# slyforce/MusicStyleTransfer

Measured on AMD Instinct MI355X. Metric: piano-roll frames/s (VAE train step), higher is better.
Workload: dtype bf16; 1 GPU; BASELINE configs[1]: single-track piano-roll VAE train step, T=256, pitch=128, latent=64, batch=64/GPU, bf16; encoder 256x2x8h, decoder 128x1x8h (scripts/train-vae.sh), dropout 0.2; Xavier-initialised weights; global_batch=64, seq_len=256, pitches=128, latent=64, parallelism=dp1, params=1885440

## Files before the change

### include/mst_hip.h

```cpp
#ifndef MST_HIP_H
#define MST_HIP_H

#include <stdint.h>

#ifdef __cplusplus
extern "C" {
#endif

typedef void* mst_stream_t;

enum mst_status {
  MST_OK = 0,
  MST_ERR_INVALID = -1,
  MST_ERR_LAUNCH = -2,
  MST_ERR_UNSUPPORTED = -3
};

enum mst_dtype { MST_BF16 = 0, MST_F16 = 1, MST_F32 = 2 };

enum mst_act { MST_ACT_NONE = 0, MST_ACT_RELU = 1 };

int mst_version(void);
const char* mst_last_error(void);

// ... 7 lines not shown
int mst_event_record(void* ev, mst_stream_t stream);
int mst_event_sync(void* ev);
int mst_event_elapsed_ms(void* ev_start, void* ev_stop, float* ms_out);
int mst_event_destroy(void* ev);

typedef struct mst_gemm_args {
  int32_t dtype;
  int32_t c_f32;
  int64_t M, N, K;
  const void* A; int64_t lda;
  const void* B; int64_t ldb;
  void* C; int64_t ldc;
  const float* bias;
  const void* resid; int64_t ldr;
  int32_t act;
  const void* gate; int64_t ldg;
  float alpha;
  const float* rowadd; int64_t ldra; int64_t rowadd_period;
  const float* grpadd; int64_t ldga; const int32_t* grp_index;
  int64_t a_rows_per_group, a_group_stride, a_group_offset;
  int64_t c_rows_per_group, c_group_stride, c_group_offset;
  float dropout_p; uint64_t dropout_seed; uint32_t dropout_site;
  int32_t self_resid;
  const uint64_t* dropout_seed_ptr;
  int32_t a_u8;
  int32_t resid_phys;
} mst_gemm_args;

int mst_gemm_nt(const mst_gemm_args* args, mst_stream_t stream);
int mst_gemm_nt_form(const mst_gemm_args* args);

int mst_gemm_nt_pair(const mst_gemm_args* args0, const mst_gemm_args* args1, mst_stream_t stream);

typedef struct mst_bce_args {
  const uint8_t* labels;
  int64_t T;
  float label_smoothing;
  int32_t downweight;
  float* loss;
  void* probs; int64_t ldp;
  void* logits; int64_t ldl;
  float gscale;
} mst_bce_args;
int mst_gemm_sigmoid_bce(const mst_gemm_args* args, const mst_bce_args* bce, mst_stream_t stream);

typedef struct mst_ln_args {
  int32_t mode;
  const float* gamma;
  const float* beta;
  float eps;
  void* out; int64_t ld_out;
  float* mean; float* rstd;
  const void* x; int64_t ld_x;
  float* dgamma; float* dbeta;
  int32_t mask_mode;
  float* partials;
} mst_ln_args;

int mst_gemm_nt_ln(const mst_gemm_args* args, const mst_ln_args* ln, mst_stream_t stream);
int mst_gemm_sigmoid_bce_dgrad_ln(const mst_gemm_args* args, const mst_bce_args* bce, const mst_gemm_args* dgrad,
                                  const mst_ln_args* ln, mst_stream_t stream);
int64_t mst_gemm_nt_ln_parts(int64_t M);
int mst_gemm_sigmoid_bce_form(const mst_gemm_args* args, const mst_bce_args* bce, const mst_gemm_args* dgrad, const mst_ln_args* ln,
                              int64_t* form);

int mst_ffn_ln_fwd(const mst_gemm_args* ff1, const mst_gemm_args* ff2, const mst_ln_args* ln, mst_stream_t stream);
int mst_ffn_ln_bwd(const mst_gemm_args* ff2_dgrad, const mst_gemm_args* ff1_dgrad, const mst_ln_args* ln, mst_stream_t stream);
typedef struct mst_ln_bwd_in {
  const void* dy; int64_t ld_dy;
  const void* x;  int64_t ld_x;
  const float* gamma; const float* mean; const float* rstd;
  void* dx; int64_t ld_dx;
  void* dx_masked; int64_t ld_dxm;
  float* dgamma; float* dbeta; float* partials;
  int32_t mask_mode;
  float dropout_p; uint64_t dropout_seed; const uint64_t* dropout_seed_ptr; uint32_t dropout_site;
} mst_ln_bwd_in;
int mst_ffn_ln_bwd_lead(const mst_ln_bwd_in* lead, const mst_gemm_args* ff2_dgrad, const mst_gemm_args* ff1_dgrad,
                        const mst_ln_args* ln, mst_stream_t stream);
int mst_proj_ffn_ln_fwd(const mst_gemm_args* proj, const mst_ln_args* ln1, const mst_gemm_args* ff1, const mst_gemm_args* ff2,
                        const mst_ln_args* ln2, mst_stream_t stream);
int mst_dec_tail_step(const mst_gemm_args* proj, const mst_ln_args* ln1, const mst_gemm_args* ff1, const mst_gemm_args* ff2,
                      const mst_ln_args* ln3, const mst_gemm_args* out, const mst_bce_args* bce, const mst_gemm_args* out_dgrad,
                      const mst_ln_args* ln3_bwd, const mst_gemm_args* ff2_dgrad, const mst_gemm_args* ff1_dgrad,
                      const mst_ln_args* ln1_bwd, mst_stream_t stream);

typedef struct mst_partial_sum {
  const float* src; int64_t n_parts; int64_t stride; int64_t len;
  float* dst; float scale;
} mst_partial_sum;
int mst_partial_sums(const mst_partial_sum* jobs, int n, mst_stream_t stream);

typedef struct mst_wgrad_args {
  int32_t dtype;
  int64_t M, N, K;
  const void* A; int64_t lda;
  const void* B; int64_t ldb;
  float* dW; int64_t ldw;
  float* db;
  float scale;
  int64_t a_rows_per_group, a_group_stride, a_group_offset;
  int64_t b_rows_per_group, b_group_stride, b_group_offset;
  int32_t a_u8;
} mst_wgrad_args;

typedef struct mst_outer_job {
  const float* L; const void* R; int32_t r_dtype; int64_t r_stride;
  int64_t B, J, I;
  float* out; float* obias;
} mst_outer_job;
int mst_outer_jobs(const mst_outer_job* jobs, int n, mst_stream_t stream);
int mst_gemm_wgrad_batch_flush(const mst_wgrad_args* list, int n, float* scratch, int64_t scratch_bytes,
                               const mst_partial_sum* sums, int n_sums, const mst_outer_job* outers, int n_outers,
                               mst_stream_t stream);
int mst_gemm_wgrad_plan(const mst_wgrad_args* list, int n, int64_t scratch_bytes, int64_t* plan);

int mst_embed_fwd(int dtype, int64_t B, int64_t T, int64_t D,
                  const int32_t* tokens, const float* table, int64_t ldt,
                  const int32_t* classes, const float* cls_table, int64_t ldc,
                  const float* pos, int64_t ldp, float alpha,
                  void* out, int64_t ld_out, int64_t S_out, int64_t s_off,
                  uint8_t* keymask, mst_stream_t stream);

int mst_embed_bwd(int dtype, int64_t B, int64_t T, int64_t D,
                  const int32_t* tokens, float* dtable, int64_t ldt,
                  const int32_t* classes, float* dcls, int64_t ldc, float alpha,
                  const void* dX, int64_t ld_dx, int64_t S_out, int64_t s_off,
                  mst_stream_t stream);

int mst_group_colsum(int dtype, int64_t B, int64_t T, int64_t D, const void* X, int64_t ldx,
                     int64_t S_out, int64_t s_off, const int32_t* idx, float* dst, int64_t ldd,
                     float alpha, mst_stream_t stream);

int mst_mask_from_lengths(int64_t B, int64_t S, const int32_t* lens, int32_t add,
                          uint8_t* keymask, mst_stream_t stream);

int mst_attn_keysoftmax_fwd(int dtype, int64_t B, int64_t S, int64_t H, int64_t dh,
                            const void* qkv, int64_t ld_qkv, int64_t k_off, int64_t q_off, int64_t v_off,
                            const uint8_t* keymask, float* lse,
                            void* out, int64_t ld_out,
                            int64_t q_limit ,
                            mst_stream_t stream);

int mst_attn_qkv_fwd(int dtype, int64_t B, int64_t S, int64_t H, int64_t dh, const void* x, int64_t ld_x, const void* w,
                     int64_t ld_w, const float* bias, void* qkv, int64_t ld_qkv, int64_t k_off, int64_t q_off, int64_t v_off,
                     const uint8_t* keymask, float* lse, void* out, int64_t ld_out, int64_t q_limit, mst_stream_t stream);
int mst_attn_keysoftmax_bwd(int dtype, int64_t B, int64_t S, int64_t H, int64_t dh,
                            const void* qkv, int64_t ld_qkv, int64_t k_off, int64_t q_off, int64_t v_off,
                            const uint8_t* keymask, const float* lse,
                            const void* dout, int64_t ld_dout,
                            void* dqkv, int64_t ld_dqkv, float* delta,
                            int64_t q_limit ,
                            mst_stream_t stream);

int mst_attn_fwd_form(int dtype, int64_t B, int64_t S, int64_t H, int64_t dh, int64_t ld_qkv, int64_t k_off, int64_t q_off,
                      int64_t v_off, int64_t ld_out, int64_t q_limit, int fused, int64_t ld_x, int64_t ld_w, int64_t* form);
int mst_attn_bwd_form(int dtype, int64_t B, int64_t S, int64_t H, int64_t dh, int64_t ld_qkv, int64_t k_off, int64_t q_off,
                      int64_t v_off, int64_t ld_dout, int64_t ld_dqkv, int64_t q_limit, int64_t* form);

int mst_attn_causal_fwd(int dtype, int64_t B, int64_t S, int64_t H, int64_t dh,
                        const void* qkv, int64_t ld_qkv, int64_t k_off, int64_t q_off, int64_t v_off,
                        const uint8_t* keymask, float* lse, void* out, int64_t ld_out, mst_stream_t stream);
int mst_attn_causal_bwd(int dtype, int64_t B, int64_t S, int64_t H, int64_t dh,
                        const void* qkv, int64_t ld_qkv, int64_t k_off, int64_t q_off, int64_t v_off,
                        const uint8_t* keymask, const float* lse, const void* dout, int64_t ld_dout,
                        void* dqkv, int64_t ld_dqkv, float* delta, mst_stream_t stream);

int mst_layernorm_fwd(int dtype, int64_t M, int64_t D, const void* x, int64_t ldx,
                      const float* gamma, const float* beta, float eps,
                      void* y, int64_t ldy, float* mean, float* rstd,
                      int64_t row_id_stride ,
                      mst_stream_t stream);

int mst_layernorm_bwd(int dtype, int64_t M, int64_t D, const void* x, int64_t ldx,
                      const float* gamma, const float* mean, const float* rstd,
                      const void* dy, int64_t ldy, void* dx, int64_t ld_dx,
                      void* dx_masked, int64_t ld_dxm, float* dgamma, float* dbeta,
                      int mask_mode, float dropout_p, uint64_t dropout_seed, uint32_t dropout_site,
                      const uint64_t* dropout_seed_ptr,
                      int64_t row_id_stride ,
                      float* partials ,
                      mst_stream_t stream);
int64_t mst_layernorm_bwd_parts(int64_t M, int64_t D);

int mst_latent_fwd(int dtype, int64_t B, int64_t De, int64_t Z, int64_t Dd,
                   const void* enc_out, int64_t enc_sample_stride,
                   const float* Wl, const float* bl, const float* eps,
                   const float* Wh, const float* bh,
                   const int32_t* classes, const float* cls_d, int64_t ld_cls,
                   const float* pos_d, float alpha_d,
                   float* mu, float* sigma, float* z, float* kl,
                   void* dec_in, int64_t dec_sample_stride, mst_stream_t stream);
int mst_latent_fwd_proj(int dtype, int64_t B, int64_t De, int64_t Z, int64_t Dd,
                        const void* enc_out, int64_t enc_sample_stride,
                        const float* Wl, const float* bl, const float* eps,
                        const float* Wh, const float* bh,
                        const int32_t* classes, const float* cls_d, int64_t ld_cls,
                        const float* pos_d, float alpha_d,
                        float* mu, float* sigma, float* z, float* kl,
                        void* dec_in, int64_t dec_sample_stride,
                        const void* Wq, int64_t ld_wq, const float* bq, void* qkv0, int64_t qkv_sample_stride, int64_t nq,
                        mst_stream_t stream);
int mst_latent_rows(int dtype, int64_t N, int64_t M, int64_t Z, int64_t Dd,
                    const float* zsrc, const float* ssrc, const int32_t* a, const int32_t* b, const float* w, int mode,
                    float tau, uint64_t seed, const uint64_t* seed_ptr, uint32_t site, int64_t row0,
                    const float* Wh, const float* bh,
                    const int32_t* ca, const int32_t* cb, const float* cw, const float* cls_d, int64_t ld_cls, int64_t n_classes,
                    const float* pos_d, float alpha_d,
                    float* z_out, void* dec_in, int64_t dec_stride, mst_stream_t stream);

int mst_latent_bwd_vec(int dtype, int64_t B, int64_t De, int64_t Z, int64_t Dd, const float* Wl, const float* eps, const float* Wh,
                       const int32_t* classes, const float* mu, const float* sigma, const void* d_dec_in, int64_t dec_sample_stride,
                       float alpha_d, float kl_weight, float gscale, float enc_scale, float* dcls_d, int64_t ld_cls,
                       void* d_enc_out, int64_t denc_sample_stride, float* scratch, mst_stream_t stream);
int mst_latent_bwd_vec_proj(int dtype, int64_t B, int64_t De, int64_t Z, int64_t Dd, const float* Wl, const float* eps, const float* Wh,
                            const int32_t* classes, const float* mu, const float* sigma,
                            const void* dq0, int64_t dq_sample_stride, const void* Wt, int64_t ld_wt, int64_t nq,
                            const void* resid0, int64_t resid_sample_stride,
                            float alpha_d, float kl_weight, float gscale, float enc_scale, float* dcls_d, int64_t ld_cls,
                            void* d_enc_out, int64_t denc_sample_stride, float* scratch, mst_stream_t stream);

int mst_latent_bwd_vec_sched(int dtype, int64_t B, int64_t De, int64_t Z, int64_t Dd, const float* Wl, const float* eps, const float* Wh,
                             const int32_t* classes, const float* mu, const float* sigma, const void* d_dec_in, int64_t dec_sample_stride,
                             float alpha_d, const float* sched, const float* kl, float gscale, float enc_scale, float* dcls_d,
                             int64_t ld_cls, void* d_enc_out, int64_t denc_sample_stride, float* scratch, mst_stream_t stream);
int mst_latent_bwd_vec_proj_sched(int dtype, int64_t B, int64_t De, int64_t Z, int64_t Dd, const float* Wl, const float* eps,
                                  const float* Wh, const int32_t* classes, const float* mu, const float* sigma,
                                  const void* dq0, int64_t dq_sample_stride, const void* Wt, int64_t ld_wt, int64_t nq,
                                  const void* resid0, int64_t resid_sample_stride,
                                  float alpha_d, const float* sched, const float* kl, float gscale, float enc_scale, float* dcls_d,
                                  int64_t ld_cls, void* d_enc_out, int64_t denc_sample_stride, float* scratch, mst_stream_t stream);

int mst_latent_form(int64_t De, int64_t Z, int64_t Dd, int64_t nq, const void* Wl, int64_t* form);

int mst_reparam_kl_fwd(int64_t B, int64_t Z, const float* mu, const float* sigma, const float* eps,
                       float* z, float* kl, mst_stream_t stream);
int mst_reparam_kl_bwd(int64_t B, int64_t Z, const float* mu, const float* sigma, const float* eps,
                       const float* dz, float kl_weight, float* dmu, float* dsigma, mst_stream_t stream);

typedef struct mst_row_tail_args {
  int32_t dtype;
  int64_t B, D;
  const void* att; int64_t rs_att;
  const void* resid; int64_t rs_res;
  const void* Wp; int64_t ldwp; const float* bp;
  const float* g1; const float* be1;
  const void* W1; int64_t ldw1; const float* b1;
  const void* W2; int64_t ldw2; const float* b2;
  const float* g2; const float* be2;
  void* h1; void* x1; void* h2; void* x2; int64_t rs_d;
  void* a; int64_t rs_a;
  float* mean1; float* rstd1; float* mean2; float* rstd2; int64_t stat_stride;
  float eps;
  float dropout_p; uint64_t dropout_seed; const uint64_t* dropout_seed_ptr; uint32_t site0;
  int64_t phys_stride;
  uint32_t* sync;
  uint32_t* status;
} mst_row_tail_args;
int mst_row_tail_fwd(const mst_row_tail_args* args, mst_stream_t stream);
int mst_row_tail_fwd_ride(const mst_row_tail_args* args, const mst_gemm_args* rider, uint32_t* queue, mst_stream_t stream);
int mst_row_tail_fwd_ride_shadows(const mst_row_tail_args* args, const mst_gemm_args* rider, uint32_t* queue, int sh_dtype,
                                  const float* sh_w, void* sh_wt16, const int64_t* sh_desc, const int64_t* sh_prefix, int64_t sh_n_mat,
                                  int64_t sh_tiles, mst_stream_t stream);
typedef struct mst_row_tail_bwd_args {
  int32_t dtype;
  int64_t B, D;
  const void* dy; int64_t rs_dy;
  const void* h2; const void* h1; int64_t rs_d;
  const void* a; int64_t rs_a;
  const float* mean1; const float* rstd1; const float* mean2; const float* rstd2; int64_t stat_stride;
  const float* g1; const float* g2;
  const void* W2t; int64_t ldw2t;
  const void* W1t; int64_t ldw1t;
  const void* Wpt; int64_t ldwpt;
  void* dh; void* dhm; void* dx1; void* dh1m; int64_t rs_c;
  void* dpre; int64_t rs_dpre;
  void* dh1; int64_t rs_dh1;
  void* datt; int64_t rs_datt;
  float* dg1; float* db1; float* dg2; float* db2;
  float dropout_p; uint64_t dropout_seed; const uint64_t* dropout_seed_ptr; uint32_t site0;
  int64_t phys_stride;
  uint32_t* sync;
  uint32_t* status;
} mst_row_tail_bwd_args;
int mst_row_tail_bwd(const mst_row_tail_bwd_args* args, mst_stream_t stream);
int mst_row_tail_bwd_ride(const mst_row_tail_bwd_args* args, const mst_gemm_args* rider, uint32_t* queue, mst_stream_t stream);
int mst_row_tail_form(int backward, int dtype, int64_t D, const mst_gemm_args* rider, int64_t sh_tiles, int64_t* form);

int mst_attn_decode(int dtype, int64_t B, int64_t H, int64_t dh, int64_t n_keys, int64_t t_max, const void* cache,
                    int64_t ld, int64_t k_off, int64_t q_off, int64_t v_off, int mode, void* out, int64_t ld_out,
                    mst_stream_t stream);

int mst_beam_step(int64_t B, int64_t K, int64_t V, int64_t i, int64_t L, const float* probs, int64_t ldp, const float* scores_in,
                  float* scores_out, const int32_t* seqs_in, int32_t* seqs_out, int32_t* hyp_src, int32_t* word, int32_t* active,
                  int32_t eos, int32_t pad, mst_stream_t stream);
int mst_beam_gather(const void* in, void* out, const int32_t* src, int64_t N, int64_t n_rows, int64_t row_bytes, int64_t t_max,
                    mst_stream_t stream);
int mst_beam_gather_cols(const void* in, void* out, const int32_t* src, int64_t N, int64_t n_rows, int64_t row_bytes, int64_t t_max,
                         int64_t skip_begin, int64_t skip_bytes, mst_stream_t stream);
int mst_sample_step(int64_t N, int64_t V, int64_t i, int64_t L, const float* probs, int64_t ldp, int32_t* seqs, float* scores,
                    int32_t* word, int32_t* active, uint64_t seed, int32_t eos, int32_t pad, mst_stream_t stream);
int mst_frame_step(int dtype, int64_t N, int64_t P, int64_t i, int64_t L, const void* logits, int64_t ldl, float tau, int mode, float thr,
                   const uint64_t* seed_ptr, uint8_t* frames, int64_t ldf, uint8_t* roll, int64_t ldr, float* scores, float* probs_out,
                   mst_stream_t stream);
int mst_token_step(int dtype, int64_t N, int64_t V, int64_t i, int64_t L, const void* logits, int64_t ldl, float tau, int32_t top_k,
                   float top_p, const uint64_t* seed_ptr, int32_t* seqs, float* scores, int32_t* word, int32_t* active,
// ... 106 lines not shown
```

### musicstyletransfer_amd/csrc/attention.hip

```cpp
#include <math.h>
#include <stdlib.h>
#include <type_traits>
#include "common.hpp"

namespace mst {

constexpr int ATT_STAGE = 64;
template <int DH> struct LdsLd { static constexpr int V = DH + 8; };
constexpr int ATT_WG_ROWS = 128;
constexpr float MASK_VALUE = -1e9f;
constexpr float NEG_BIG = -3.0e38f;
constexpr float LOG2E = 1.4426950408889634f;

__device__ __forceinline__ void key_consts(bool in_range, bool valid_key, float rmax, float logl, float scale, float& sk2,
                                           float& ck2) {
  if (!in_range) { sk2 = 0.f; ck2 = -INFINITY; }
  else if (!valid_key) { sk2 = 0.f; ck2 = -logl * LOG2E; }
  else { sk2 = scale * LOG2E; ck2 = -(rmax + logl) * LOG2E; }
}
__device__ __forceinline__ float fast_exp2(float x) { return __builtin_amdgcn_exp2f(x); }
#define MST_FOR_TILES(kt, bits) for (uint64_t mst_m_ = (bits); mst_m_; mst_m_ &= mst_m_ - 1) if (const int kt = __builtin_ctzll(mst_m_); true)
__device__ __forceinline__ uint64_t tile_bits(int n) { return n >= 64 ? ~0ull : ((1ull << n) - 1ull); }
__device__ __forceinline__ uint64_t padded_tile_mask(const float* sSk, const float* sCk, int n_tiles, int lane) {
  uint32_t lo = 0u, hi = 0u;
// ... 887 lines not shown
        a.lse[plane + bh * S + k_lane] = logl;
      }
      key_consts(in, vk, in ? M : 0.f, in ? logl : 0.f, a.scale, sSk[k_lane], sCk[k_lane]);
      sMadd[k_lane] = madd; sMax[k_lane] = in ? M : 0.f; sLogl[k_lane] = in ? logl : INFINITY;
    }
    padded |= (in && !vk);
  }
  if constexpr (DH <= 16) {
    if (lone) {
      const int64_t e = S - 1;
      const bool vk = a.keymask[b * S + e];
      const float madd = vk ? 0.f : MASK_VALUE;
      float ke[DH];
      if (restage) {
#pragma unroll
        for (int f = 0; f < DH; ++f) ke[f] = to_f32(base[a.k_off + e * a.ld_qkv + f]);
      } else {
        lds_row_load<T, DH>(sK + e * LD, ke);
      }
      float m = NEG_BIG, l = 0.f;
      for (int q = tid; q < S; q += nthr) {
        const float t = fmaf(lds_row_dot<T, DH>(sQ + q * LD, ke), a.scale, madd);
        const float m_new = fmaxf(m, t);
        l = l * __expf(m - m_new) + __expf(t - m_new);
        m = m_new;
      }
      const float mw = wave_max(m);
      const float lw = wave_sum(l * __expf(m - mw));
      if (lane == 0) { sRed[wave] = mw; sRed[16 + wave] = lw; }
      __syncthreads();
      if (tid == 0) {
        float M = NEG_BIG, L = 0.f;
        for (int w = 0; w < NW; ++w) M = fmaxf(M, sRed[w]);
        for (int w = 0; w < NW; ++w) L += sRed[16 + w] * __expf(sRed[w] - M);
        const float logl = __logf(L);
        a.lse[bh * S + e] = M;
        a.lse[plane + bh * S + e] = logl;
        key_consts(true, vk, M, logl, a.scale, sSk[e], sCk[e]);
        sMadd[e] = madd; sMax[e] = M; sLogl[e] = logl;
        for (int k = (int)S; k < SP; ++k) { key_consts(false, false, 0.f, 0.f, a.scale, sSk[k], sCk[k]); sMadd[k] = MASK_VALUE; sMax[k] = 0.f; sLogl[k] = INFINITY; }
      }
      padded |= !vk;
    }
  }
  const bool exact = __syncthreads_or(padded);
  const uint64_t pad_tiles = exact ? padded_tile_mask(sSk, sCk, NB, lane) : 0ull;
  ATT_STAMP(3);
  if constexpr (CHUNKED) {
    constexpr int OBM = 2;
    typename Act<T>::vec8 qf[OBM][KS];
    f32x16 o[OBM][DB];
    bool act[OBM];
#pragma unroll
    for (int i = 0; i < OBM; ++i) {
      const int ob = wave + i * NW;
      act[i] = ob < NBo && (int64_t)ob * 32 < a.q_limit;
#pragma unroll
      for (int s = 0; s < KS; ++s) qf[i][s] = glb_row_frag<T>(base + a.q_off, a.ld_qkv, act[i] ? (int64_t)ob * 32 + (lane & 31) : S, S, s, lane);
#pragma unroll
      for (int d = 0; d < DB; ++d) o[i][d] = zero16<DH>();
    }
    const int tiles_c = CR / 32;
    for (int c = 0; c < a.restage; ++c) {
      if (c > 0) __syncthreads();
      const int64_t k0 = (int64_t)c * CR;
      stage_pair<T, DH>(sK, base + a.k_off + k0 * a.ld_qkv, a.ld_qkv, S - k0, sV, base + a.v_off + k0 * a.ld_qkv, a.ld_qkv, S - k0, CR, tid, nthr);
      __syncthreads();
      const int nt = (NBo - c * tiles_c) < tiles_c ? (NBo - c * tiles_c) : tiles_c;
#pragma unroll
      for (int i = 0; i < OBM; ++i) {
        if (!act[i]) continue;
        if (exact) {
          const uint64_t padc = (pad_tiles >> (c * tiles_c)) & tile_bits(nt);
          MST_FOR_TILES(kt, ~padc & tile_bits(nt)) fwd_out_tile<T, DH, false>(sK, sV, sSk + k0, sCk + k0, sMadd + k0, sMax + k0, sLogl + k0, kt, a.scale, qf[i], o[i], lane);
          MST_FOR_TILES(kt, padc) fwd_out_tile<T, DH, true>(sK, sV, sSk + k0, sCk + k0, sMadd + k0, sMax + k0, sLogl + k0, kt, a.scale, qf[i], o[i], lane);
        } else {
          for (int kt = 0; kt < nt; ++kt) fwd_out_tile<T, DH, false>(sK, sV, sSk + k0, sCk + k0, sMadd + k0, sMax + k0, sLogl + k0, kt, a.scale, qf[i], o[i], lane);
        }
      }
    }
    T* og = reinterpret_cast<T*>(a.out) + b * S * a.ld_out + hd * DH;
#pragma unroll
    for (int i = 0; i < OBM; ++i) {
      const int64_t q_lane = (int64_t)(wave + i * NW) * 32 + (lane & 31);
      owner_store<T, DH>((act[i] && q_lane < S && q_lane < a.q_limit) ? og + q_lane * a.ld_out : nullptr, o[i], lane);
    }
    return;
  }
  if (restage) {
    stage_pair<T, DH>(sK, base + a.k_off, a.ld_qkv, S, sV, base + a.v_off, a.ld_qkv, S, SP, tid, nthr);
    __syncthreads();
  }

  for (int ob = wave; ob < NBo; ob += NW) {
    if ((int64_t)ob * 32 >= a.q_limit) break;
    typename Act<T>::vec8 qf[KS];
#pragma unroll
    for (int s = 0; s < KS; ++s)
      qf[s] = restage ? glb_row_frag<T>(base + a.q_off, a.ld_qkv, (int64_t)ob * 32 + (lane & 31), S, s, lane) : lds_row_frag<T, DH>(sQ, ob * 32, s, lane);
    f32x16 o[DB];
#pragma unroll
    for (int d = 0; d < DB; ++d) o[d] = zero16<DH>();
    if (exact) {
      MST_FOR_TILES(kt, ~pad_tiles & tile_bits(NBo)) fwd_out_tile<T, DH, false>(sK, sV, sSk, sCk, sMadd, sMax, sLogl, kt, a.scale, qf, o, lane);
      MST_FOR_TILES(kt, pad_tiles & tile_bits(NBo)) fwd_out_tile<T, DH, true>(sK, sV, sSk, sCk, sMadd, sMax, sLogl, kt, a.scale, qf, o, lane);
    } else {
      for (int kt = 0; kt < NBo; ++kt) fwd_out_tile<T, DH, false>(sK, sV, sSk, sCk, sMadd, sMax, sLogl, kt, a.scale, qf, o, lane);
    }
    if constexpr (DH <= 16) {
      if (lone) {
        if (exact) fwd_out_tile<T, DH, true, true>(sK, sV, sSk, sCk, sMadd, sMax, sLogl, NB - 1, a.scale, qf, o, lane);
        else fwd_out_tile<T, DH, false, true>(sK, sV, sSk, sCk, sMadd, sMax, sLogl, NB - 1, a.scale, qf, o, lane);
      }
    }
    T* og = reinterpret_cast<T*>(a.out) + b * S * a.ld_out + hd * DH;
    const int64_t q_lane = ob * 32 + (lane & 31);
    owner_store<T, DH>((q_lane < S && q_lane < a.q_limit) ? og + q_lane * a.ld_out : nullptr, o, lane);
  }
  ATT_STAMP(4);
  if constexpr (DH <= 16) {
    if (lone) {
      const int64_t e = S - 1;
      float qe[DH], acc[DH];
      if (restage) {
#pragma unroll
        for (int f = 0; f < DH; ++f) qe[f] = to_f32(base[a.q_off + e * a.ld_qkv + f]);
      } else {
        lds_row_load<T, DH>(sQ + e * LD, qe);
      }
#pragma unroll
      for (int f = 0; f < DH; ++f) acc[f] = 0.f;
      for (int k = tid; k < S; k += nthr) {
        const float x = lds_row_dot<T, DH>(sK + k * LD, qe);
        const float p = exact ? exact_prob(x, a.scale, sMadd[k], sMax[k], sLogl[k]) : fast_exp2(fmaf(x, sSk[k], sCk[k]));
        lds_row_axpy<T, DH>(p, sV + k * LD, acc);
      }
#pragma unroll
      for (int f = 0; f < DH; ++f) acc[f] = wave_sum(acc[f]);
      if (lane == 0) {
#pragma unroll
        for (int f = 0; f < DH; ++f) sRed[wave * DH + f] = acc[f];
      }
      __syncthreads();
      if (tid < DH) {
        float o_e = 0.f;
        for (int w = 0; w < NW; ++w) o_e += sRed[w * DH + tid];
        T* og = reinterpret_cast<T*>(a.out) + b * S * a.ld_out + hd * DH;
        og[e * a.ld_out + tid] = (T)o_e;
      }
    }
  }
}

template <typename T, int DH, bool SPARSE>
__global__ __launch_bounds__(RES_MAX_WAVES<DH> * 64) __attribute__((amdgpu_waves_per_eu(DH == 16 ? ATT16_WAVES : (DH == 64 ? 2 : 4)))) void attn_bwd_res_kernel(AttnArgs a) {
  constexpr int KS = DH / 16, DB = (DH + 31) / 32, LD = LdsLd<DH>::V;
  extern __shared__ __attribute__((aligned(16))) unsigned char att_smem[];
  const int64_t S = a.S;
  const int NB = (int)((S + 31) / 32), SP = NB * 32;
  T* bufA = reinterpret_cast<T*>(att_smem);
  T* bufB = bufA + SP * LD;
  float* sSk = reinterpret_cast<float*>(bufB + SP * LD);
  float* sCk = sSk + SP; float* sMadd = sCk + SP; float* sMax = sMadd + SP; float* sLogl = sMax + SP; float* sNd = sLogl + SP;
  float* sRed = sNd + SP;
  const int tid = threadIdx.x, lane = tid & 63, wave = tid >> 6, nthr = blockDim.x, NW = nthr >> 6;
  const int64_t bh = res_wg_bh(a.B, a.H), b = (int64_t)((uint32_t)bh / (uint32_t)a.H), hd = bh - b * a.H;
  const int64_t plane = a.B * a.H * S;
  const bool lone = !SPARSE && lone_row_shape(S, DH);
  const int NBo = lone ? NB - 1 : NB;
  const float log2_scale = __log2f(a.scale);
  const T* base = reinterpret_cast<const T*>(a.qkv) + b * S * a.ld_qkv + hd * DH;
  const T* Kg = base + a.k_off;
  const T* Qg = base + a.q_off;
  const T* Vg = base + a.v_off;
  const T* dOg = reinterpret_cast<const T*>(a.dout) + b * S * a.ld_dout + hd * DH;
  T* dbase = reinterpret_cast<T*>(a.dqkv) + b * S * a.ld_dqkv + hd * DH;
  constexpr bool sparse = SPARSE;
  const int64_t do_rows = sparse ? a.q_limit : S;
  typename Act<T>::vec8 kf[KS], vf[KS];
#pragma unroll
  for (int s = 0; s < KS; ++s) {
    kf[s] = glb_row_frag<T>(Kg, a.ld_qkv, wave * 32 + (lane & 31), S, s, lane);
    vf[s] = glb_row_frag<T>(Vg, a.ld_qkv, wave * 32 + (lane & 31), S, s, lane);
  }
  ATT_STAMP(0);
  stage_pair<T, DH>(bufA, Qg, a.ld_qkv, S, bufB, dOg, a.ld_dout, do_rows, SP, tid, nthr);
  __syncthreads();
  ATT_STAMP(1);
  const int nq0 = sparse ? 1 : NBo;

  int padded = 0;
  for (int ob = wave; ob < NBo; ob += NW) {
    const int64_t k_lane = ob * 32 + (lane & 31);
    if (ob != wave) {
#pragma unroll
      for (int s = 0; s < KS; ++s) {
        kf[s] = glb_row_frag<T>(Kg, a.ld_qkv, k_lane, S, s, lane);
        vf[s] = glb_row_frag<T>(Vg, a.ld_qkv, k_lane, S, s, lane);
      }
    }
    const bool in = k_lane < S;
    const bool vk = in && a.keymask[b * S + k_lane];
    const float rmax = in ? a.lse[bh * S + k_lane] : 0.f;
    const float logl = in ? a.lse[plane + bh * S + k_lane] : INFINITY;
    const float madd = vk ? 0.f : MASK_VALUE;
    float sk2, ck2;
    key_consts(in, vk, rmax, in ? logl : 0.f, a.scale, sk2, ck2);
    const float ck2s = ck2 + log2_scale;
    const bool exact_w = __any(in && !vk);
    padded |= (in && !vk);
    f32x16 acc[DB];
    float neg_delta = 0.f;
    T* const drow = in ? dbase + k_lane * a.ld_dqkv : nullptr;
#pragma unroll
    for (int d = 0; d < DB; ++d) acc[d] = zero16<DH>();
    if (exact_w) for (int qt = 0; qt < nq0; ++qt) bwd_kv_tile<T, DH, 0, true>(bufA, bufB, qt, a.scale, kf, vf, sk2, ck2, madd, rmax, logl, neg_delta, acc, lane);
    else for (int qt = 0; qt < nq0; ++qt) bwd_kv_tile<T, DH, 0, false>(bufA, bufB, qt, a.scale, kf, vf, sk2, ck2, madd, rmax, logl, neg_delta, acc, lane);
    if constexpr (DH <= 16 && !SPARSE) {
      if (lone) {
        if (exact_w) bwd_kv_tile<T, DH, 0, true, false, true>(bufA, bufB, NB - 1, a.scale, kf, vf, sk2, ck2, madd, rmax, logl, neg_delta, acc, lane);
        else bwd_kv_tile<T, DH, 0, false, false, true>(bufA, bufB, NB - 1, a.scale, kf, vf, sk2, ck2, madd, rmax, logl, neg_delta, acc, lane);
      }
    }
    {
      const float delta = delta_from_dv<T, DH>(acc, vf, lane);
      if (lane < 32 && in) a.delta[bh * S + k_lane] = delta;
      neg_delta = -delta;
    }
    owner_store<T, DH>(drow ? drow + a.v_off : nullptr, acc, lane);
    ATT_STAMP(2);
#pragma unroll
    for (int d = 0; d < DB; ++d) acc[d] = zero16<DH>();
    if (exact_w) for (int qt = 0; qt < nq0; ++qt) bwd_kv_tile<T, DH, 1, true>(bufA, bufB, qt, a.scale, kf, vf, sk2, ck2s, madd, rmax, logl, neg_delta, acc, lane);
    else for (int qt = 0; qt < nq0; ++qt) bwd_kv_tile<T, DH, 1, false>(bufA, bufB, qt, a.scale, kf, vf, sk2, ck2s, madd, rmax, logl, neg_delta, acc, lane);
    if (sparse) {
      if (exact_w) for (int qt = nq0; qt < NB; ++qt) bwd_kv_tile<T, DH, 1, true, true>(bufA, bufB, qt, a.scale, kf, vf, sk2, ck2s, madd, rmax, logl, neg_delta, acc, lane);
      else for (int qt = nq0; qt < NB; ++qt) bwd_kv_tile<T, DH, 1, false, true>(bufA, bufB, qt, a.scale, kf, vf, sk2, ck2s, madd, rmax, logl, neg_delta, acc, lane);
    }
    if constexpr (DH <= 16 && !SPARSE) {
      if (lone) {
        if (exact_w) bwd_kv_tile<T, DH, 1, true, false, true>(bufA, bufB, NB - 1, a.scale, kf, vf, sk2, ck2s, madd, rmax, logl, neg_delta, acc, lane);
        else bwd_kv_tile<T, DH, 1, false, false, true>(bufA, bufB, NB - 1, a.scale, kf, vf, sk2, ck2s, madd, rmax, logl, neg_delta, acc, lane);
      }
    }
    owner_store<T, DH>(drow ? drow + a.k_off : nullptr, acc, lane);
    if (lane < 32) {
      sSk[k_lane] = sk2; sCk[k_lane] = ck2s; sMadd[k_lane] = madd; sMax[k_lane] = rmax; sLogl[k_lane] = logl;
      sNd[k_lane] = in ? neg_delta : 0.f;
    }
  }
  if constexpr (DH <= 16 && !SPARSE) {
    if (lone) {
      const int64_t e = S - 1;
      float ke[DH], ve[DH], acc[DH];
#pragma unroll
      for (int f = 0; f < DH; ++f) { ke[f] = to_f32(Kg[e * a.ld_qkv + f]); ve[f] = to_f32(Vg[e * a.ld_qkv + f]); }
      const bool vk = a.keymask[b * S + e];
      const float rmax = a.lse[bh * S + e], logl = a.lse[plane + bh * S + e], madd = vk ? 0.f : MASK_VALUE;
      float sk2, ck2;
      key_consts(true, vk, rmax, logl, a.scale, sk2, ck2);
      const float ck2s = ck2 + log2_scale;
      padded |= !vk;
#pragma unroll
      for (int f = 0; f < DH; ++f) acc[f] = 0.f;
      for (int q = tid; q < S; q += nthr) {
        const float x = lds_row_dot<T, DH>(bufA + q * LD, ke);
        const float pr = vk ? fast_exp2(fmaf(x, sk2, ck2)) : exact_prob(x, a.scale, madd, rmax, logl);
        lds_row_axpy<T, DH>(pr, bufB + q * LD, acc);
      }
#pragma unroll
      for (int f = 0; f < DH; ++f) acc[f] = wave_sum(acc[f]);
      if (lane == 0) {
#pragma unroll
        for (int f = 0; f < DH; ++f) sRed[wave * DH + f] = acc[f];
      }
      __syncthreads();
      if (tid < DH) {
        float dv = 0.f;
        for (int w = 0; w < NW; ++w) dv += sRed[w * DH + tid];
        sRed[LONE_RED / 2 + tid] = dv;
        dbase[e * a.ld_dqkv + a.v_off + tid] = (T)dv;
      }
      __syncthreads();
      float delta = 0.f;
#pragma unroll
      for (int f = 0; f < DH; ++f) delta = fmaf(ve[f], sRed[LONE_RED / 2 + f], delta);
#pragma unroll
      for (int f = 0; f < DH; ++f) acc[f] = 0.f;
      for (int q = tid; q < S; q += nthr) {
        const float x = lds_row_dot<T, DH>(bufA + q * LD, ke);
        const float ps = vk ? fast_exp2(fmaf(x, sk2, ck2s)) : exact_prob(x, a.scale, madd, rmax, logl) * a.scale;
        const float dl = ps * (lds_row_dot<T, DH>(bufB + q * LD, ve) - delta);
        lds_row_axpy<T, DH>(dl, bufA + q * LD, acc);
      }
#pragma unroll
      for (int f = 0; f < DH; ++f) acc[f] = wave_sum(acc[f]);
      __syncthreads();
      if (lane == 0) {
#pragma unroll
        for (int f = 0; f < DH; ++f) sRed[wave * DH + f] = acc[f];
      }
      __syncthreads();
      if (tid < DH) {
        float dk = 0.f;
        for (int w = 0; w < NW; ++w) dk += sRed[w * DH + tid];
        dbase[e * a.ld_dqkv + a.k_off + tid] = (T)dk;
      }
      if (tid == 0) {
        a.delta[bh * S + e] = delta;
        sSk[e] = sk2; sCk[e] = ck2s; sMadd[e] = madd; sMax[e] = rmax; sLogl[e] = logl; sNd[e] = -delta;
        for (int k = (int)S; k < SP; ++k) {
          float s0, c0;
          key_consts(false, false, 0.f, 0.f, a.scale, s0, c0);
          sSk[k] = s0; sCk[k] = c0 + log2_scale; sMadd[k] = MASK_VALUE; sMax[k] = 0.f; sLogl[k] = INFINITY; sNd[k] = 0.f;
        }
      }
    }
  }
  ATT_STAMP(3);
  typename Act<T>::vec8 qf[KS], dof[KS];
#pragma unroll
  for (int s = 0; s < KS; ++s) {
    qf[s] = glb_row_frag<T>(Qg, a.ld_qkv, wave * 32 + (lane & 31), S, s, lane);
    dof[s] = glb_row_frag<T>(dOg, a.ld_dout, wave * 32 + (lane & 31), do_rows, s, lane);
  }
  __syncthreads();
  stage_pair<T, DH>(bufA, Kg, a.ld_qkv, S, bufB, Vg, a.ld_qkv, S, SP, tid, nthr);
  const bool exact = __syncthreads_or(padded);
  const uint64_t pad_tiles = exact ? padded_tile_mask(sSk, sCk, NB, lane) : 0ull;
  ATT_STAMP(4);

  for (int ob = wave; ob < NBo; ob += NW) {
    const int64_t q_lane = ob * 32 + (lane & 31);
    if (ob != wave) {
#pragma unroll
      for (int s = 0; s < KS; ++s) {
        qf[s] = glb_row_frag<T>(Qg, a.ld_qkv, q_lane, S, s, lane);
        dof[s] = glb_row_frag<T>(dOg, a.ld_dout, q_lane, do_rows, s, lane);
      }
    }
    f32x16 acc[DB];
#pragma unroll
    for (int d = 0; d < DB; ++d) acc[d] = zero16<DH>();
    if (sparse && ob > 0) {
      if (exact) {
        MST_FOR_TILES(kt, ~pad_tiles & tile_bits(NB)) bwd_q_tile<T, DH, false, true>(bufA, bufB, sSk, sCk, sMadd, sMax, sLogl, sNd, kt, a.scale, qf, dof, acc, lane);
        MST_FOR_TILES(kt, pad_tiles & tile_bits(NB)) bwd_q_tile<T, DH, true, true>(bufA, bufB, sSk, sCk, sMadd, sMax, sLogl, sNd, kt, a.scale, qf, dof, acc, lane);
      } else for (int kt = 0; kt < NB; ++kt) bwd_q_tile<T, DH, false, true>(bufA, bufB, sSk, sCk, sMadd, sMax, sLogl, sNd, kt, a.scale, qf, dof, acc, lane);
    } else if (exact) {
      MST_FOR_TILES(kt, ~pad_tiles & tile_bits(NBo)) bwd_q_tile<T, DH, false>(bufA, bufB, sSk, sCk, sMadd, sMax, sLogl, sNd, kt, a.scale, qf, dof, acc, lane);
      MST_FOR_TILES(kt, pad_tiles & tile_bits(NBo)) bwd_q_tile<T, DH, true>(bufA, bufB, sSk, sCk, sMadd, sMax, sLogl, sNd, kt, a.scale, qf, dof, acc, lane);
    } else {
      for (int kt = 0; kt < NBo; ++kt) bwd_q_tile<T, DH, false>(bufA, bufB, sSk, sCk, sMadd, sMax, sLogl, sNd, kt, a.scale, qf, dof, acc, lane);
    }
    if constexpr (DH <= 16 && !SPARSE) {
      if (lone) {
        if (exact) bwd_q_tile<T, DH, true, false, true>(bufA, bufB, sSk, sCk, sMadd, sMax, sLogl, sNd, NB - 1, a.scale, qf, dof, acc, lane);
        else bwd_q_tile<T, DH, false, false, true>(bufA, bufB, sSk, sCk, sMadd, sMax, sLogl, sNd, NB - 1, a.scale, qf, dof, acc, lane);
      }
    }
    owner_store<T, DH>(q_lane < S ? dbase + a.q_off + q_lane * a.ld_dqkv : nullptr, acc, lane);
  }
  ATT_STAMP(5);
  if constexpr (DH <= 16 && !SPARSE) {
    if (lone) {
      const int64_t e = S - 1;
      float qe[DH], doe[DH], acc[DH];
#pragma unroll
      for (int f = 0; f < DH; ++f) { qe[f] = to_f32(Qg[e * a.ld_qkv + f]); doe[f] = to_f32(dOg[e * a.ld_dout + f]); acc[f] = 0.f; }
      for (int k = tid; k < S; k += nthr) {
        const float x = lds_row_dot<T, DH>(bufA + k * LD, qe);
        const float ps = exact ? exact_prob(x, a.scale, sMadd[k], sMax[k], sLogl[k]) * a.scale : fast_exp2(fmaf(x, sSk[k], sCk[k]));
        const float dl = ps * (lds_row_dot<T, DH>(bufB + k * LD, doe) + sNd[k]);
        lds_row_axpy<T, DH>(dl, bufA + k * LD, acc);
      }
#pragma unroll
      for (int f = 0; f < DH; ++f) acc[f] = wave_sum(acc[f]);
      if (lane == 0) {
#pragma unroll
        for (int f = 0; f < DH; ++f) sRed[wave * DH + f] = acc[f];
      }
      __syncthreads();
      if (tid < DH) {
        float dq = 0.f;
        for (int w = 0; w < NW; ++w) dq += sRed[w * DH + tid];
        dbase[e * a.ld_dqkv + a.q_off + tid] = (T)dq;
      }
    }
  }
}

template <typename T, int DH, int OBM>
__global__ __launch_bounds__(512) void attn_bwd_q_chunk_kernel(AttnArgs a, int n_chunks) {
  constexpr int KS = DH / 16, DB = (DH + 31) / 32, LD = LdsLd<DH>::V;
  extern __shared__ __attribute__((aligned(16))) unsigned char att_smem[];
  const int64_t S = a.S;
  const int NB = (int)((S + 31) / 32), SP = NB * 32, CR = SP / n_chunks;
  T* sK = reinterpret_cast<T*>(att_smem);
  T* sV = sK + CR * LD;
  float* sSk = reinterpret_cast<float*>(sV + CR * LD);
  float* sCk = sSk + SP; float* sMadd = sCk + SP; float* sMax = sMadd + SP; float* sLogl = sMax + SP; float* sNd = sLogl + SP;
  const int tid = threadIdx.x, lane = tid & 63, wave = tid >> 6, nthr = blockDim.x, NW = nthr >> 6;
  const int64_t bh = res_wg_bh(a.B, a.H), b = (int64_t)((uint32_t)bh / (uint32_t)a.H), hd = bh - b * a.H;
  const int64_t plane = a.B * a.H * S;
  const float log2_scale = __log2f(a.scale);
  const T* base = reinterpret_cast<const T*>(a.qkv) + b * S * a.ld_qkv + hd * DH;
  const T* dOg = reinterpret_cast<const T*>(a.dout) + b * S * a.ld_dout + hd * DH;
  const bool sparse = a.q_limit > 0 && a.q_limit <= 32;
  const int64_t do_rows = sparse ? a.q_limit : S;
  typename Act<T>::vec8 qf[OBM][KS], dof[OBM][KS];
  f32x16 acc[OBM][DB];
  bool act[OBM];
#pragma unroll
  for (int i = 0; i < OBM; ++i) {
    const int ob = wave + i * NW;
    act[i] = ob < NB;
    const int64_t q_lane = act[i] ? (int64_t)ob * 32 + (lane & 31) : S;
#pragma unroll
    for (int s = 0; s < KS; ++s) {
      qf[i][s] = glb_row_frag<T>(base + a.q_off, a.ld_qkv, q_lane, S, s, lane);
      dof[i][s] = glb_row_frag<T>(dOg, a.ld_dout, q_lane, do_rows, s, lane);
    }
#pragma unroll
    for (int d = 0; d < DB; ++d) acc[i][d] = zero16<DH>();
  }
  int padded = 0;
  for (int k = tid; k < SP; k += nthr) {
    const bool in = k < S;
    const bool vk = in && a.keymask[b * S + k];
    const float rmax = in ? a.lse[bh * S + k] : 0.f, logl = in ? a.lse[plane + bh * S + k] : 0.f;
    float sk2, ck2;
    key_consts(in, vk, rmax, logl, a.scale, sk2, ck2);
    sSk[k] = sk2; sCk[k] = ck2 + log2_scale;
    sMadd[k] = vk ? 0.f : MASK_VALUE; sMax[k] = rmax; sLogl[k] = in ? logl : INFINITY;
    sNd[k] = in ? -a.delta[bh * S + k] : 0.f;
    padded |= (in && !vk);
  }
  const bool exact = __syncthreads_or(padded);
  const uint64_t pad_tiles = exact ? padded_tile_mask(sSk, sCk, NB, lane) : 0ull;
  const int tiles_c = CR / 32;
  for (int c = 0; c < n_chunks; ++c) {
    if (c > 0) __syncthreads();
    const int64_t k0 = (int64_t)c * CR;
    if (k0 >= S) break;
    stage_pair<T, DH>(sK, base + a.k_off + k0 * a.ld_qkv, a.ld_qkv, S - k0, sV, base + a.v_off + k0 * a.ld_qkv, a.ld_qkv, S - k0, CR, tid, nthr);
    __syncthreads();
    const int nt = (NB - c * tiles_c) < tiles_c ? (NB - c * tiles_c) : tiles_c;
#pragma unroll
    for (int i = 0; i < OBM; ++i) {
      if (!act[i]) continue;
      const bool light = sparse && (wave + i * NW) > 0;
      if (light) {
        if (exact) {
          const uint64_t padc = (pad_tiles >> (c * tiles_c)) & tile_bits(nt);
          MST_FOR_TILES(kt, ~padc & tile_bits(nt)) bwd_q_tile<T, DH, false, true>(sK, sV, sSk + k0, sCk + k0, sMadd + k0, sMax + k0, sLogl + k0, sNd + k0, kt, a.scale, qf[i], dof[i], acc[i], lane);
          MST_FOR_TILES(kt, padc) bwd_q_tile<T, DH, true, true>(sK, sV, sSk + k0, sCk + k0, sMadd + k0, sMax + k0, sLogl + k0, sNd + k0, kt, a.scale, qf[i], dof[i], acc[i], lane);
        } else for (int kt = 0; kt < nt; ++kt) bwd_q_tile<T, DH, false, true>(sK, sV, sSk + k0, sCk + k0, sMadd + k0, sMax + k0, sLogl + k0, sNd + k0, kt, a.scale, qf[i], dof[i], acc[i], lane);
      } else if (exact) {
        const uint64_t padc = (pad_tiles >> (c * tiles_c)) & tile_bits(nt);
        MST_FOR_TILES(kt, ~padc & tile_bits(nt)) bwd_q_tile<T, DH, false>(sK, sV, sSk + k0, sCk + k0, sMadd + k0, sMax + k0, sLogl + k0, sNd + k0, kt, a.scale, qf[i], dof[i], acc[i], lane);
        MST_FOR_TILES(kt, padc) bwd_q_tile<T, DH, true>(sK, sV, sSk + k0, sCk + k0, sMadd + k0, sMax + k0, sLogl + k0, sNd + k0, kt, a.scale, qf[i], dof[i], acc[i], lane);
      } else {
        for (int kt = 0; kt < nt; ++kt) bwd_q_tile<T, DH, false>(sK, sV, sSk + k0, sCk + k0, sMadd + k0, sMax + k0, sLogl + k0, sNd + k0, kt, a.scale, qf[i], dof[i], acc[i], lane);
      }
    }
  }
  T* dst = reinterpret_cast<T*>(a.dqkv) + b * S * a.ld_dqkv + hd * DH + a.q_off;
#pragma unroll
  for (int i = 0; i < OBM; ++i) {
    const int64_t q_lane = (int64_t)(wave + i * NW) * 32 + (lane & 31);
    owner_store<T, DH>((act[i] && q_lane < S) ? dst + q_lane * a.ld_dqkv : nullptr, acc[i], lane);
  }
}

static int choose_resident(int64_t S, int64_t n_wg, size_t lds_bytes, int waves_cu = 16, bool lone = false, int max_nw = 16) {
  const char* force = getenv("MST_ATTN_PATH");
  if (force && force[0] == 's') return 0;
  const size_t LDS_CU = 160 * 1024;
  if (lds_bytes > LDS_CU - 1024) return 0;
  const int NB = (int)cdiv(S, 32) - (lone ? 1 : 0);
  const int by_grid = (int)cdiv(n_wg, 256);
  int best = 0;
  double best_score = 0.0;
  for (int nw = 1; nw <= max_nw && nw <= NB; ++nw) {
    int wgs = waves_cu / nw;
    if ((size_t)wgs * lds_bytes > LDS_CU) wgs = (int)(LDS_CU / lds_bytes);
    if (wgs > by_grid) wgs = by_grid;
    if (wgs < 1) continue;
    const double eff = (double)NB / (double)(nw * cdiv(NB, nw));
    const double score = (double)(wgs * nw) * eff;
    if (score >= best_score) { best_score = score; best = nw; }
  }
  return best;
}
static size_t res_lds_fwd(int dh, int64_t S, int tiles) { const size_t SP = (size_t)cdiv(S, 32) * 32; return (size_t)tiles * SP * (dh + 8) * 2 + 5 * SP * 4 + LONE_RED * 4; }
static size_t res_lds_bwd(int dh, int64_t S) { const size_t SP = (size_t)cdiv(S, 32) * 32; return 2 * SP * (dh + 8) * 2 + 6 * SP * 4 + LONE_RED * 4; }
static int res_max_waves(int dh) { return dh == 64 ? RES_MAX_WAVES<64> : RES_MAX_WAVES<32>; }

static int attn_check(int64_t B, int64_t S, int64_t H, int64_t dh, int64_t ld, int64_t k_off, int64_t q_off, int64_t v_off) {
  MST_CHECK_ARG(B > 0 && S > 0 && H > 0, "attention: B,S,H must be positive");
  MST_CHECK_ARG(dh == 16 || dh == 32 || dh == 64, "attention: head size must be 16, 32 or 64 (got %lld)", (long long)dh);
  MST_CHECK_ARG(ld % 8 == 0 && k_off % 8 == 0 && q_off % 8 == 0 && v_off % 8 == 0, "attention: ld and offsets must be multiples of 8");
  MST_CHECK_ARG(B * H <= 65535, "attention: B*H too large for grid.y");
  return MST_OK;
}
static int attn_check_fwd(int64_t B, int64_t S, int64_t H, int64_t dh, int64_t ld_qkv, int64_t k_off, int64_t q_off, int64_t v_off, int64_t ld_out) {
  const int rc = attn_check(B, S, H, dh, ld_qkv, k_off, q_off, v_off);
  if (rc) return rc;
  MST_CHECK_ARG(ld_out >= H * dh, "mst_attn_keysoftmax_fwd: ld_out < H*dh");
  return MST_OK;
}
static int attn_check_qkv(int64_t B, int64_t S, int64_t H, int64_t dh, int64_t ld_x, int64_t ld_w, int64_t ld_qkv, int64_t k_off, int64_t q_off,
                          int64_t v_off, int64_t ld_out) {
  const int rc = attn_check(B, S, H, dh, ld_qkv, k_off, q_off, v_off);
  if (rc) return rc;
  const int64_t Dm = H * dh;
  MST_CHECK_ARG(ld_x % 8 == 0 && ld_x >= Dm && ld_w % 8 == 0 && ld_w >= Dm && ld_qkv >= 3 * Dm && ld_out >= Dm,
                "mst_attn_qkv_fwd: leading dimensions must be multiples of 8 and cover the model width");
  MST_CHECK_ARG(k_off + Dm <= 3 * Dm && q_off + Dm <= 3 * Dm && v_off + Dm <= 3 * Dm, "mst_attn_qkv_fwd: section offsets beyond the 3 D weight rows");
  return MST_OK;
}
static int attn_check_bwd(int64_t B, int64_t S, int64_t H, int64_t dh, int64_t ld_qkv, int64_t k_off, int64_t q_off, int64_t v_off, int64_t ld_dout,
                          int64_t ld_dqkv) {
  const int rc = attn_check(B, S, H, dh, ld_qkv, k_off, q_off, v_off);
  if (rc) return rc;
  MST_CHECK_ARG(ld_dout % 8 == 0 && ld_dout >= H * dh && ld_dqkv % 8 == 0, "mst_attn_keysoftmax_bwd: bad leading dims");
  return MST_OK;
}
static int check_act_dtype(int dtype) { return dispatch_act(dtype, [](auto) -> int { return MST_OK; }); }
static int64_t fwd_q_limit(int64_t q_limit, int64_t S) { return (q_limit > 0 && q_limit < S) ? q_limit : S; }
static int64_t bwd_q_limit(int64_t q_limit, int64_t S) { return (q_limit > 0 && q_limit < S) ? q_limit : 0; }

enum { ATT_FWD_RES3 = 0, ATT_FWD_RES2 = 1, ATT_FWD_CHUNKED = 2, ATT_FWD_FUSED = 3, ATT_FWD_STREAM = 4 };
enum { ATT_BWD_RES = 0, ATT_BWD_STREAM_CHUNKQ = 1, ATT_BWD_STREAM = 2 };
struct AttnFwdForm { int path, waves; size_t lds; int lone, restage; int64_t grid_stats, grid_out; };
struct AttnBwdForm { int path, waves; size_t lds; int sparse, lone, dq_chunks, dq_waves; };
constexpr int ATT_DQ_OBM = 4, ATT_DQ_NW = 8;

static AttnFwdForm attn_fwd_form(int dh, int64_t S, int64_t H, int64_t n_wg, int64_t q_limit, bool fused_call) {
  AttnFwdForm f = {};
  const int NB = (int)cdiv(S, 32);
  if (fused_call && dh == 32) {
    const int64_t Dm = H * dh;
    const size_t lds = res_lds_fwd(32, S, 3);
    const int nw = choose_resident(S, n_wg, lds, 16, false);
    if (nw >= NB && nw >= 6 && Dm % QKV_KC == 0) { f.path = ATT_FWD_FUSED; f.waves = nw; f.lds = lds; return f; }
  }
  const bool lone = lone_row_shape(S, dh) && q_limit >= S;
  const int waves_cu = dh == 16 ? 4 * ATT16_WAVES : 16;
  f.lone = lone;
  for (int tiles = 3; tiles >= 2; --tiles) {
    const size_t lds = res_lds_fwd(dh, S, tiles);
    if (const int nw = choose_resident(S, n_wg, lds, waves_cu, lone)) {
      f.path = tiles == 3 ? ATT_FWD_RES3 : ATT_FWD_RES2; f.waves = nw; f.lds = lds; f.restage = tiles == 3 ? 0 : 1;
      return f;
    }
  }
  if (!lone && dh >= 32 && NB % 2 == 0) {
    const size_t lds = res_lds_fwd(dh, S, 1);
    const int maxw = res_max_waves(dh);
    const int nw = choose_resident(S, n_wg, lds, maxw, false, maxw);
    if (nw && NB <= 2 * nw) { f.path = ATT_FWD_CHUNKED; f.waves = nw; f.lds = lds; f.restage = 2; return f; }
  }
  f.path = ATT_FWD_STREAM; f.waves = 4; f.lone = 0;
  f.grid_stats = cdiv(S, ATT_WG_ROWS); f.grid_out = cdiv(q_limit, ATT_WG_ROWS);
  return f;
}
static AttnBwdForm attn_bwd_form(int dh, int64_t S, int64_t n_wg, int64_t q_limit) {
  AttnBwdForm f = {};
  f.sparse = q_limit > 0 && q_limit <= 32;
  const bool lone = lone_row_shape(S, dh) && !f.sparse;
  const size_t lds = res_lds_bwd(dh, S);
  if (const int nw = choose_resident(S, n_wg, lds, dh == 16 ? 4 * ATT16_WAVES : res_max_waves(dh), lone, res_max_waves(dh))) {
    f.path = ATT_BWD_RES; f.waves = nw; f.lds = lds; f.lone = lone;
    return f;
  }
  f.path = ATT_BWD_STREAM; f.waves = 4;
  const int NB = (int)cdiv(S, 32);
  if (dh == 32 && NB <= ATT_DQ_OBM * ATT_DQ_NW) {
    for (int nc = 1; nc <= 4; nc *= 2) {
      if (NB % nc != 0) break;
      const size_t lds_q = (size_t)2 * (NB * 32 / nc) * (dh + 8) * 2 + (size_t)6 * NB * 32 * 4;
      if (lds_q > 150 * 1024) continue;
      f.path = ATT_BWD_STREAM_CHUNKQ; f.lds = lds_q; f.dq_chunks = nc; f.dq_waves = ATT_DQ_NW;
      break;
    }
  }
  return f;
}

template <typename T, int DH>
static int launch_fwd(const AttnArgs& a_in, const AttnFwdForm& f, hipStream_t s) {
  AttnArgs a = a_in;
  a.restage = f.restage;
  const dim3 grid_res((unsigned)(a.B * a.H)), block_res(f.waves * 64);
  switch (f.path) {
    case ATT_FWD_FUSED: {
      if constexpr (DH == 32) {
        static size_t granted = 64 * 1024;
        if (const int rc = lds_opt_in(reinterpret_cast<const void*>(&attn_fwd_res_kernel<T, DH, true>), f.lds, &granted, "attn_fwd_res_kernel (fused projection)")) return rc;
        hipLaunchKernelGGL((attn_fwd_res_kernel<T, DH, true>), grid_res, block_res, f.lds, s, a);
        MST_CHECK_LAUNCH("attn_fwd_res_kernel (fused projection)");
        return MST_OK;
      }
      break;
    }
    case ATT_FWD_CHUNKED: {
      if (DH >= 32) {
        static size_t granted = 64 * 1024;
        if (const int rc = lds_opt_in(reinterpret_cast<const void*>(&attn_fwd_res_kernel<T, DH, false, true>), f.lds, &granted, "attn_fwd_res_kernel (chunked)")) return rc;
        hipLaunchKernelGGL((attn_fwd_res_kernel<T, DH, false, true>), grid_res, block_res, f.lds, s, a);
        MST_CHECK_LAUNCH("attn_fwd_res_kernel (chunked)");
        return MST_OK;
      }
      break;
    }
    case ATT_FWD_RES3:
    case ATT_FWD_RES2: {
      static size_t granted = 64 * 1024;
      if (const int rc = lds_opt_in(reinterpret_cast<const void*>(&attn_fwd_res_kernel<T, DH>), f.lds, &granted, "attn_fwd_res_kernel")) return rc;
      hipLaunchKernelGGL((attn_fwd_res_kernel<T, DH>), grid_res, block_res, f.lds, s, a);
      MST_CHECK_LAUNCH("attn_fwd_res_kernel");
      return MST_OK;
    }
    case ATT_FWD_STREAM: {
      const dim3 grid((unsigned)f.grid_stats, (unsigned)(a.B * a.H));
      hipLaunchKernelGGL((attn_fwd_stats_kernel<T, DH>), grid, dim3(256), 0, s, a);
      MST_CHECK_LAUNCH("attn_fwd_stats_kernel");
      const dim3 grid_o((unsigned)f.grid_out, (unsigned)(a.B * a.H));
      hipLaunchKernelGGL((attn_fwd_out_kernel<T, DH>), grid_o, dim3(256), 0, s, a);
      MST_CHECK_LAUNCH("attn_fwd_out_kernel");
      return MST_OK;
    }
  }
  set_error("attention forward: form %d has no kernel at head size %d", f.path, DH);
  return MST_ERR_INVALID;
}
template <typename T, int DH>
static int launch_bwd(const AttnArgs& a, const AttnBwdForm& f, hipStream_t s) {
  if (f.path == ATT_BWD_RES) {
    static size_t granted[2] = {64 * 1024, 64 * 1024};
    const void* fn = f.sparse ? reinterpret_cast<const void*>(&attn_bwd_res_kernel<T, DH, true>)
                              : reinterpret_cast<const void*>(&attn_bwd_res_kernel<T, DH, false>);
    if (const int rc = lds_opt_in(fn, f.lds, &granted[f.sparse], "attn_bwd_res_kernel")) return rc;
    if (f.sparse) hipLaunchKernelGGL((attn_bwd_res_kernel<T, DH, true>), dim3((unsigned)(a.B * a.H)), dim3(f.waves * 64), f.lds, s, a);
    else hipLaunchKernelGGL((attn_bwd_res_kernel<T, DH, false>), dim3((unsigned)(a.B * a.H)), dim3(f.waves * 64), f.lds, s, a);
    MST_CHECK_LAUNCH("attn_bwd_res_kernel");
    return MST_OK;
  }
  const dim3 grid((unsigned)cdiv(a.S, ATT_WG_ROWS), (unsigned)(a.B * a.H));
  if (f.sparse) hipLaunchKernelGGL((attn_bwd_kv_kernel<T, DH, true>), grid, dim3(256), 0, s, a);
  else hipLaunchKernelGGL((attn_bwd_kv_kernel<T, DH, false>), grid, dim3(256), 0, s, a);
  MST_CHECK_LAUNCH("attn_bwd_kv_kernel");
  if (f.path == ATT_BWD_STREAM_CHUNKQ) {
    if (DH == 32) {
      static size_t granted = 64 * 1024;
      if (const int rc = lds_opt_in(reinterpret_cast<const void*>(&attn_bwd_q_chunk_kernel<T, DH, ATT_DQ_OBM>), f.lds, &granted, "attn_bwd_q_chunk_kernel")) return rc;
      hipLaunchKernelGGL((attn_bwd_q_chunk_kernel<T, DH, ATT_DQ_OBM>), dim3((unsigned)(a.B * a.H)), dim3(f.dq_waves * 64), f.lds, s, a, f.dq_chunks);
      MST_CHECK_LAUNCH("attn_bwd_q_chunk_kernel");
      return MST_OK;
    }
    set_error("attention backward: chunked dQ has no kernel at head size %d", DH);
    return MST_ERR_INVALID;
  }
  hipLaunchKernelGGL((attn_bwd_q_kernel<T, DH>), grid, dim3(256), 0, s, a);
  MST_CHECK_LAUNCH("attn_bwd_q_kernel");
  return MST_OK;
}
template <typename T>
static int launch_fwd_dh(int64_t dh, const AttnArgs& a, const AttnFwdForm& f, hipStream_t s) {
  if (dh == 16) return launch_fwd<T, 16>(a, f, s);
  if (dh == 32) return launch_fwd<T, 32>(a, f, s);
  return launch_fwd<T, 64>(a, f, s);
}


template <typename T, int DH>
__global__ __launch_bounds__(64) void attn_decode_kernel(int64_t H, int64_t n_keys, int64_t t_max, const T* __restrict__ cache,
                                                          int64_t ld, int64_t k_off, int64_t q_off, int64_t v_off, int mode,
                                                          float scale, T* __restrict__ out, int64_t ld_out) {
  const int64_t b = blockIdx.x / H, hd = blockIdx.x % H;
  const int lane = threadIdx.x;
  const T* base = cache + b * t_max * ld + hd * DH;
  float q[DH];
#pragma unroll
  for (int d = 0; d < DH; ++d) q[d] = to_f32(base[(n_keys - 1) * ld + q_off + d]);
  float m = -INFINITY;
  if (mode == 1) {
    for (int64_t k = lane; k < n_keys; k += 64) {
      float l = 0.f;
#pragma unroll
      for (int d = 0; d < DH; ++d) l = fmaf(to_f32(base[k * ld + k_off + d]), q[d], l);
      m = fmaxf(m, l * scale);
    }
    m = wave_max(m);
  }
  float acc[DH], z = 0.f;
#pragma unroll
  for (int d = 0; d < DH; ++d) acc[d] = 0.f;
  for (int64_t k = lane; k < n_keys; k += 64) {
    float p = 1.f;
    if (mode == 1) {
      float l = 0.f;
#pragma unroll
      for (int d = 0; d < DH; ++d) l = fmaf(to_f32(base[k * ld + k_off + d]), q[d], l);
      p = __expf(l * scale - m);
    }
    z += p;
#pragma unroll
    for (int d = 0; d < DH; ++d) acc[d] = fmaf(p, to_f32(base[k * ld + v_off + d]), acc[d]);
  }
  z = wave_sum(z);
  const float inv = (mode == 1) ? 1.f / z : 1.f;
#pragma unroll
  for (int d = 0; d < DH; ++d) {
    const float v = wave_sum(acc[d]);
    if (lane == 0) out[b * ld_out + hd * DH + d] = from_f32<T>(v * inv);
  }
}

}

using namespace mst;

extern "C" int mst_attn_keysoftmax_fwd(int dtype, int64_t B, int64_t S, int64_t H, int64_t dh, const void* qkv,
                                       int64_t ld_qkv, int64_t k_off, int64_t q_off, int64_t v_off,
                                       const uint8_t* keymask, float* lse, void* out, int64_t ld_out,
                                       int64_t q_limit, mst_stream_t stream) {
  int rc = attn_check(B, S, H, dh, ld_qkv, k_off, q_off, v_off);
  if (rc) return rc;
  MST_CHECK_ARG(qkv && keymask && lse && out, "mst_attn_keysoftmax_fwd: null pointer");
  rc = attn_check_fwd(B, S, H, dh, ld_qkv, k_off, q_off, v_off, ld_out);
  if (rc) return rc;
  AttnArgs a = {};
  a.B = B; a.S = S; a.H = H; a.qkv = qkv; a.ld_qkv = ld_qkv; a.k_off = k_off; a.q_off = q_off; a.v_off = v_off;
  a.keymask = keymask; a.lse = lse; a.out = out; a.ld_out = ld_out;
  a.q_limit = fwd_q_limit(q_limit, S);
  a.scale = 1.f / sqrtf((float)dh);
  hipStream_t s = (hipStream_t)stream;
  return dispatch_act(dtype, [&](auto tag) -> int {
    return launch_fwd_dh<decltype(tag)>(dh, a, attn_fwd_form((int)dh, S, H, B * H, a.q_limit, false), s);
  });
}

static void put_fwd_form(const AttnFwdForm& f, int64_t* form) {
  const int64_t v[8] = {f.path, f.waves, (int64_t)f.lds, f.lone, f.grid_stats, f.grid_out, 0, 0};
  for (int i = 0; i < 8; ++i) form[i] = v[i];
}
extern "C" int mst_attn_fwd_form(int dtype, int64_t B, int64_t S, int64_t H, int64_t dh, int64_t ld_qkv, int64_t k_off, int64_t q_off,
                                 int64_t v_off, int64_t ld_out, int64_t q_limit, int fused, int64_t ld_x, int64_t ld_w, int64_t* form) {
  MST_CHECK_ARG(form != nullptr, "mst_attn_fwd_form: null form");
  int rc = fused ? attn_check_qkv(B, S, H, dh, ld_x, ld_w, ld_qkv, k_off, q_off, v_off, ld_out)
                 : attn_check_fwd(B, S, H, dh, ld_qkv, k_off, q_off, v_off, ld_out);
  if (rc == MST_OK) rc = check_act_dtype(dtype);
  if (rc) return rc;
  put_fwd_form(attn_fwd_form((int)dh, S, H, B * H, fwd_q_limit(q_limit, S), fused != 0), form);
  return MST_OK;
}
extern "C" int mst_attn_bwd_form(int dtype, int64_t B, int64_t S, int64_t H, int64_t dh, int64_t ld_qkv, int64_t k_off, int64_t q_off,
                                 int64_t v_off, int64_t ld_dout, int64_t ld_dqkv, int64_t q_limit, int64_t* form) {
  MST_CHECK_ARG(form != nullptr, "mst_attn_bwd_form: null form");
  int rc = attn_check_bwd(B, S, H, dh, ld_qkv, k_off, q_off, v_off, ld_dout, ld_dqkv);
  if (rc == MST_OK) rc = check_act_dtype(dtype);
  if (rc) return rc;
  const AttnBwdForm f = attn_bwd_form((int)dh, S, B * H, bwd_q_limit(q_limit, S));
  const int64_t v[8] = {f.path, f.waves, (int64_t)f.lds, f.sparse, f.lone, f.dq_chunks, f.dq_waves, 0};
  for (int i = 0; i < 8; ++i) form[i] = v[i];
  return MST_OK;
}

#ifdef MST_ATT_STAMPS
extern "C" int mst_debug_att_loop(uint64_t* host_out) {
  return hipMemcpyFromSymbol(host_out, HIP_SYMBOL(mst::g_att_loop), sizeof(uint64_t) * 256) == hipSuccess ? 0 : -1;
}
extern "C" int mst_debug_att_stamps(uint64_t* host_out) {
  return hipMemcpyFromSymbol(host_out, HIP_SYMBOL(mst::g_att_stamps), sizeof(uint64_t) * 8192) == hipSuccess ? 0 : -1;
}
#endif

extern "C" int mst_attn_qkv_fwd(int dtype, int64_t B, int64_t S, int64_t H, int64_t dh, const void* x, int64_t ld_x, const void* w,
                                int64_t ld_w, const float* bias, void* qkv, int64_t ld_qkv, int64_t k_off, int64_t q_off, int64_t v_off,
                                const uint8_t* keymask, float* lse, void* out, int64_t ld_out, int64_t q_limit, mst_stream_t stream) {
  int rc = attn_check_qkv(B, S, H, dh, ld_x, ld_w, ld_qkv, k_off, q_off, v_off, ld_out);
  if (rc) return rc;
  const int64_t Dm = H * dh;
  MST_CHECK_ARG(x && w && bias && qkv && keymask && lse && out, "mst_attn_qkv_fwd: null pointer");
  MST_CHECK_ARG(((uintptr_t)x % 16 == 0) && ((uintptr_t)w % 16 == 0) && ((uintptr_t)bias % 16 == 0) && ((uintptr_t)qkv % 16 == 0),
                "mst_attn_qkv_fwd: operands must be 16-byte aligned");
  rc = check_act_dtype(dtype);
  if (rc) return rc;
  AttnArgs a = {};
  a.B = B; a.S = S; a.H = H; a.qkv = qkv; a.ld_qkv = ld_qkv; a.k_off = k_off; a.q_off = q_off; a.v_off = v_off;
  a.keymask = keymask; a.lse = lse; a.out = out; a.ld_out = ld_out;
  a.q_limit = fwd_q_limit(q_limit, S);
  a.scale = 1.f / sqrtf((float)dh);
  const AttnFwdForm f = attn_fwd_form((int)dh, S, H, B * H, a.q_limit, true);
  if (f.path == ATT_FWD_FUSED) {
    a.x = x; a.ld_x = ld_x; a.w = w; a.ld_w = ld_w; a.bias = bias; a.Dm = Dm;
  } else {
    mst_gemm_args g = {};
    g.dtype = dtype; g.M = B * S; g.N = 3 * Dm; g.K = Dm;
    g.A = x; g.lda = ld_x; g.B = w; g.ldb = ld_w; g.C = qkv; g.ldc = ld_qkv; g.bias = bias; g.alpha = 1.f;
    rc = mst_gemm_nt(&g, stream);
    if (rc) return rc;
  }
  hipStream_t s = (hipStream_t)stream;
  return dispatch_act(dtype, [&](auto tag) -> int { return launch_fwd_dh<decltype(tag)>(dh, a, f, s); });
}

extern "C" int mst_attn_keysoftmax_bwd(int dtype, int64_t B, int64_t S, int64_t H, int64_t dh, const void* qkv,
                                       int64_t ld_qkv, int64_t k_off, int64_t q_off, int64_t v_off,
                                       const uint8_t* keymask, const float* lse, const void* dout, int64_t ld_dout,
                                       void* dqkv, int64_t ld_dqkv, float* delta, int64_t q_limit, mst_stream_t stream) {
  int rc = attn_check(B, S, H, dh, ld_qkv, k_off, q_off, v_off);
  if (rc) return rc;
  MST_CHECK_ARG(qkv && keymask && lse && dout && dqkv && delta, "mst_attn_keysoftmax_bwd: null pointer");
  rc = attn_check_bwd(B, S, H, dh, ld_qkv, k_off, q_off, v_off, ld_dout, ld_dqkv);
  if (rc) return rc;
  AttnArgs a = {};
  a.B = B; a.S = S; a.H = H; a.qkv = qkv; a.ld_qkv = ld_qkv; a.k_off = k_off; a.q_off = q_off; a.v_off = v_off;
  a.keymask = keymask; a.lse = const_cast<float*>(lse); a.dout = dout; a.ld_dout = ld_dout; a.dqkv = dqkv;
  a.ld_dqkv = ld_dqkv; a.delta = delta;
  a.q_limit = bwd_q_limit(q_limit, S);
  a.scale = 1.f / sqrtf((float)dh);
  hipStream_t s = (hipStream_t)stream;
  return dispatch_act(dtype, [&](auto tag) -> int {
    typedef decltype(tag) T;
    const AttnBwdForm f = attn_bwd_form((int)dh, S, B * H, a.q_limit);
    if (dh == 16) return launch_bwd<T, 16>(a, f, s);
    if (dh == 32) return launch_bwd<T, 32>(a, f, s);
    return launch_bwd<T, 64>(a, f, s);
  });
}

extern "C" int mst_attn_decode(int dtype, int64_t B, int64_t H, int64_t dh, int64_t n_keys, int64_t t_max, const void* cache,
                               int64_t ld, int64_t k_off, int64_t q_off, int64_t v_off, int mode, void* out, int64_t ld_out,
                               mst_stream_t stream) {
  MST_CHECK_ARG(B > 0 && H > 0 && n_keys > 0 && n_keys <= t_max && cache && out, "mst_attn_decode: bad argument");
  MST_CHECK_ARG(dh == 16 || dh == 32 || dh == 64, "mst_attn_decode: head size must be 16, 32 or 64 (got %lld)", (long long)dh);
  MST_CHECK_ARG(mode == 0 || mode == 1, "mst_attn_decode: mode must be 0 (softmax over the query axis, the reference) or 1 (over the keys)");
  MST_CHECK_ARG(ld_out >= H * dh, "mst_attn_decode: ld_out < H*dh");
  const float scale = 1.f / sqrtf((float)dh);
  hipStream_t s = (hipStream_t)stream;
  return dispatch_act(dtype, [&](auto tag) -> int {
    typedef decltype(tag) T;
    const dim3 grid((unsigned)(B * H));
    if (dh == 16) hipLaunchKernelGGL((attn_decode_kernel<T, 16>), grid, dim3(64), 0, s, H, n_keys, t_max, (const T*)cache, ld, k_off, q_off, v_off, mode, scale, (T*)out, ld_out);
    else if (dh == 32) hipLaunchKernelGGL((attn_decode_kernel<T, 32>), grid, dim3(64), 0, s, H, n_keys, t_max, (const T*)cache, ld, k_off, q_off, v_off, mode, scale, (T*)out, ld_out);
    else hipLaunchKernelGGL((attn_decode_kernel<T, 64>), grid, dim3(64), 0, s, H, n_keys, t_max, (const T*)cache, ld, k_off, q_off, v_off, mode, scale, (T*)out, ld_out);
    MST_CHECK_LAUNCH("attn_decode_kernel");
    return MST_OK;
  });
}
```

### musicstyletransfer_amd/csrc/runtime.hip

```cpp
#include <stdarg.h>
#include <string.h>
#include "common.hpp"

namespace mst {
static thread_local char g_err[512] = "";
void set_error(const char* fmt, ...) {
  va_list ap;
  va_start(ap, fmt);
  vsnprintf(g_err, sizeof(g_err), fmt, ap);
  va_end(ap);
}
}

using namespace mst;

extern "C" int mst_version(void) { return 112; }
extern "C" const char* mst_last_error(void) { return g_err; }

#define HIP_TRY(expr)                                             \
  do {                                                            \
    hipError_t e__ = (expr);                                      \
    if (e__ != hipSuccess) {                                      \
      set_error("%s: %s", #expr, hipGetErrorString(e__));         \
      return MST_ERR_LAUNCH;                                      \
    }                                                             \
  } while (0)

extern "C" int mst_graph_begin(mst_stream_t stream) {
  HIP_TRY(hipStreamBeginCapture((hipStream_t)stream, hipStreamCaptureModeThreadLocal));
  return MST_OK;
}
static hipError_t count_nodes(hipGraph_t g, int32_t* nodes_out, int32_t* kernel_nodes_out) {
  size_t n = 0;
  hipError_t e = hipGraphGetNodes(g, nullptr, &n);
  if (e != hipSuccess) return e;
  int32_t kernels = 0;
  if (n > 0 && kernel_nodes_out) {
    hipGraphNode_t* nodes = new hipGraphNode_t[n];
    e = hipGraphGetNodes(g, nodes, &n);
    for (size_t i = 0; e == hipSuccess && i < n; ++i) {
      hipGraphNodeType t;
      e = hipGraphNodeGetType(nodes[i], &t);
      kernels += (e == hipSuccess && t == hipGraphNodeTypeKernel);
    }
    delete[] nodes;
    if (e != hipSuccess) return e;
  }
  if (nodes_out) *nodes_out = (int32_t)n;
  if (kernel_nodes_out) *kernel_nodes_out = kernels;
  return hipSuccess;
}

extern "C" int mst_graph_end(mst_stream_t stream, void** graph_exec_out) {
  return mst_graph_end_counted(stream, graph_exec_out, nullptr, nullptr);
}
extern "C" int mst_graph_end_counted(mst_stream_t stream, void** graph_exec_out, int32_t* nodes_out, int32_t* kernel_nodes_out) {
  MST_CHECK_ARG(graph_exec_out != nullptr, "mst_graph_end: null output");
  hipGraph_t g = nullptr;
  HIP_TRY(hipStreamEndCapture((hipStream_t)stream, &g));
  hipError_t ec = (nodes_out || kernel_nodes_out) ? count_nodes(g, nodes_out, kernel_nodes_out) : hipSuccess;
  if (ec != hipSuccess) {
    (void)hipGraphDestroy(g);
    set_error("hipGraphGetNodes: %s", hipGetErrorString(ec));
    return MST_ERR_LAUNCH;
  }
  hipGraphExec_t ge = nullptr;
  hipError_t e = hipGraphInstantiate(&ge, g, nullptr, nullptr, 0);
  (void)hipGraphDestroy(g);
  if (e != hipSuccess) {
    set_error("hipGraphInstantiate: %s", hipGetErrorString(e));
    return MST_ERR_LAUNCH;
  }
  *graph_exec_out = (void*)ge;
  return MST_OK;
}
extern "C" int mst_graph_launch(void* graph_exec, mst_stream_t stream) {
  HIP_TRY(hipGraphLaunch((hipGraphExec_t)graph_exec, (hipStream_t)stream));
  return MST_OK;
}
extern "C" int mst_graph_destroy(void* graph_exec) {
  if (graph_exec) HIP_TRY(hipGraphExecDestroy((hipGraphExec_t)graph_exec));
  return MST_OK;
}

extern "C" int mst_event_create(void** ev_out) {
  MST_CHECK_ARG(ev_out != nullptr, "mst_event_create: null output");
  hipEvent_t ev;
  HIP_TRY(hipEventCreate(&ev));
  *ev_out = (void*)ev;
  return MST_OK;
}
extern "C" int mst_event_record(void* ev, mst_stream_t stream) {
  HIP_TRY(hipEventRecord((hipEvent_t)ev, (hipStream_t)stream));
  return MST_OK;
}
extern "C" int mst_event_sync(void* ev) {
  HIP_TRY(hipEventSynchronize((hipEvent_t)ev));
  return MST_OK;
}
extern "C" int mst_event_elapsed_ms(void* a, void* b, float* ms_out) {
  HIP_TRY(hipEventElapsedTime(ms_out, (hipEvent_t)a, (hipEvent_t)b));
  return MST_OK;
}
extern "C" int mst_event_destroy(void* ev) {
  if (ev) HIP_TRY(hipEventDestroy((hipEvent_t)ev));
  return MST_OK;
}

__global__ void selftest_kernel(int32_t* flags) {
  __shared__ __bf16 tile[32 * 32];
  const int l = threadIdx.x;
  auto Aval = [](int i, int k) { return (float)(((i * 3 + k * 5) % 7) - 3); };
  auto Bval = [](int k, int j) { return (float)(((k * 2 + j * 7) % 5) - 2); };

  {
    bf16x8 a, b;
    for (int j = 0; j < 8; ++j) {
      a[j] = (__bf16)Aval(l & 15, 8 * (l >> 4) + j);
      b[j] = (__bf16)Bval(8 * (l >> 4) + j, l & 15);
    }
    f32x4 d = {0, 0, 0, 0};
    d = __builtin_amdgcn_mfma_f32_16x16x32_bf16(a, b, d, 0, 0, 0);
    int ok = 1;
    for (int r = 0; r < 4; ++r) {
      int row = 4 * (l >> 4) + r, col = l & 15;
      float ref = 0;
      for (int k = 0; k < 32; ++k) ref += Aval(row, k) * Bval(k, col);
      ok &= (d[r] == ref);
    }
    ok = __all(ok);
    if (l == 0) flags[0] = ok;
  }
  f32x16 X;
  {
    bf16x8 a, b;
    for (int j = 0; j < 8; ++j) {
      a[j] = (__bf16)Aval(l & 31, 8 * (l >> 5) + j);
      b[j] = (__bf16)Bval(8 * (l >> 5) + j, l & 31);
    }
    f32x16 d;
    for (int r = 0; r < 16; ++r) d[r] = 0;
    d = __builtin_amdgcn_mfma_f32_32x32x16_bf16(a, b, d, 0, 0, 0);
    int ok = 1;
    for (int r = 0; r < 16; ++r) {
      int row = (r & 3) + 8 * (r >> 2) + 4 * (l >> 5), col = l & 31;
      float ref = 0;
      for (int k = 0; k < 16; ++k) ref += Aval(row, k) * Bval(k, col);
      ok &= (d[r] == ref);
    }
    ok = __all(ok);
    if (l == 0) flags[1] = ok;
    X = d;
  }
  auto Tval = [](int r, int c) { return (float)((r * 37 + c * 11) % 251); };
  for (int i = l; i < 32 * 32; i += 64) tile[i] = (__bf16)Tval(i / 32, i % 32);
  __syncthreads();
  {
    int g_i = l & 15, q = g_i >> 2, p = g_i & 3;
    int r0 = 8 + 4 * (l >> 5), c0 = 16 * ((l >> 4) & 1);
    const __bf16* addr = &tile[(r0 + q) * 32 + c0 + 4 * p];
    i16x4 v = __builtin_amdgcn_ds_read_tr16_b64_v4i16(
        (__attribute__((address_space(3))) i16x4*)(uintptr_t)(addr));
    int ok = 1;
    for (int e = 0; e < 4; ++e) {
      uint16_t bits = (uint16_t)v[e];
      float got = bits_to_f32<__bf16>(bits);
      ok &= (got == Tval(r0 + e, c0 + g_i));
    }
    ok = __all(ok);
// ... 38 lines not shown
```

### musicstyletransfer_amd/engine.py

```python
import contextlib
import math
import os
import warnings
from collections import OrderedDict, namedtuple

import numpy as np
import torch

from . import ops as o
from ._lib import CE_MAX_WORKGROUPS
from .ops import roundup


class VAEConfig:

    def __init__(self, kind, in_dim, out_dim, num_classes, latent_dim, e_model, e_layers, e_heads, d_model, d_layers,
                 d_heads, e_dropout=0.0, d_dropout=0.0, d_causal=False):
        assert kind in ("token", "pianoroll")
        assert e_model % e_heads == 0 and d_model % d_heads == 0
        self.kind = kind
        self.in_dim, self.out_dim = in_dim, out_dim
        self.num_classes, self.latent_dim = num_classes, latent_dim
        self.e_model, self.e_layers, self.e_heads = e_model, e_layers, e_heads
        self.d_model, self.d_layers, self.d_heads = d_model, d_layers, d_heads
# ... 293 lines not shown
        return flat[off: off + 3 * D * D].view(3 * D, D) if what == "weight" else flat[off: off + 3 * D]

    def t(self, name):
        so, r, c = self.t_specs[name]
        off = self.t_off[name]
        return self.wt16[off: off + c * roundup(r, 8)].view(c, roundup(r, 8))

    def _layer_params(self, side, i):
        pre = f"{side}.layer{i}"

        def dense(name):
            w, b = f"{pre}.{name}.weight", f"{pre}.{name}.bias"
            return Dense(self.h(w), self.p(b), self.t(w), self.grad(w), self.grad(b))

        def norm(name):
            g, b = f"{pre}.{name}.gamma", f"{pre}.{name}.beta"
            return Norm(self.p(g), self.p(b), self.grad(g), self.grad(b), f"{pre}.{name}")

        kqv = Dense(self.fused(self.w16, pre, "weight"), self.fused(self.w, pre, "bias"), self.t(f"{pre}.att.W_kqv"),
                    self.fused(self.g, pre, "weight"), self.fused(self.g, pre, "bias"))
        dec = side == "decoder"
        return LayerParams(kqv, dense("att.W_proj"), dense("ff1"), dense("ff2"), norm("ln1"), norm("ln3" if dec else "ln2"),
                           self_resid=dec, mask_mode=2 if dec else 1)

    def layer(self, side, i):
        return self._layers[side, i]

    def load_numpy(self, params_np):
        host = np.zeros(self.n, np.float32)
        for name, shape in self.shapes.items():
            a = np.asarray(params_np[name], np.float32)
            assert tuple(a.shape) == tuple(shape), f"{name}: expected {shape}, got {a.shape}"
            host[self.offsets[name]: self.offsets[name] + a.size] = a.reshape(-1)
        self.w.copy_(torch.from_numpy(host))
        self.refresh_shadows()

    def to_numpy(self, which="w"):
        if which == "ema" and self.ema is None:
            raise RuntimeError("this store keeps no average of its weights (StepPlan(ema_decay=...) / enable_ema())")
        host = getattr(self, which).detach().cpu().numpy()
        return OrderedDict((n, host[self.offsets[n]: self.offsets[n] + int(np.prod(s))].reshape(s).copy())
                           for n, s in self.shapes.items())

    def shadowed_names(self):
        names = set()
        for key in self.t_specs:
            if key.endswith(".att.W_kqv"):
                p = key[: -len("W_kqv")]
                names.update({p + "W_k.weight", p + "W_q.weight", p + "W_v.weight"})
            else:
                names.add(key)
        return names

    def as_consumed_numpy(self):
        w = self.to_numpy("w")
        w16 = self.w16.detach().float().cpu().numpy()
        for n in self.shadowed_names():
            s = self.shapes[n]
            w[n] = w16[self.offsets[n]: self.offsets[n] + int(np.prod(s))].reshape(s).copy()
        return w

    def load_ema_numpy(self, params_np=None):
        self.enable_ema()
        if params_np is None:
            self.ema.copy_(self.w)
            return
        host = np.zeros(self.n, np.float32)
        for name, shape in self.shapes.items():
            a = np.asarray(params_np[name], np.float32)
            assert tuple(a.shape) == tuple(shape), f"{name}: expected {shape}, got {a.shape}"
            host[self.offsets[name]: self.offsets[name] + a.size] = a.reshape(-1)
        self.ema.copy_(torch.from_numpy(host))

    def refresh_shadows(self):
        o.cast_to_act(self.w, self.w16)
        o.transpose_shadows(self.w, self.wt16, self.t_desc, self.t_prefix, len(self.t_specs), self.t_tiles)


class _Layer:
    pass


Dense = namedtuple("Dense", "w b t dw db")
Norm = namedtuple("Norm", "gamma beta dgamma dbeta site")
LayerParams = namedtuple("LayerParams", "kqv proj ff1 ff2 ln1 ln2 self_resid mask_mode")

Rows = namedtuple("Rows", "view c_remap ln")
ALL_ROWS = Rows(lambda buf: buf, (0, 0, 0), {})


def position0_rows(B, S):
    return Rows(lambda buf: buf.view(B, S, -1)[:, 0, :], (1, S, 0), dict(M=B, row_id_stride=S))


class Dropout(namedtuple("Dropout", "p seed_ptr site0")):

    def at(self, k):
        return dict(dropout_p=self.p, dropout_site=self.site0 + k, dropout_seed_ptr=self.seed_ptr) if self.p > 0 else {}


NO_DROPOUT = Dropout(0.0, None, 0)


def row_block_fwd(P, L, x_in, rows, drop, form, row_groups=None, tail=None, launch=True):
    D, v = P.proj.w.shape[0], rows.view
    if form == "tail":
        o.row_tail_fwd(v(L.att), v(x_in), P.proj.w, P.proj.b, P.ln1.gamma, P.ln1.beta, P.ff1.w, P.ff1.b, P.ff2.w, P.ff2.b, P.ln2.gamma,
                       P.ln2.beta, v(L.h1), v(L.x1), v(L.a), v(L.h2), v(L.x2), L.mean1, L.rstd1, L.mean2, L.rstd2, dropout_p=drop.p,
                       dropout_seed_ptr=drop.seed_ptr, site0=drop.site0, **tail)
        return L.x2
    proj = dict(N=D, K=D, bias=P.proj.b, resid=v(x_in), **drop.at(0))
    ff1 = dict(K=D, bias=P.ff1.b, act=o.ACT_RELU, **drop.at(1))
    ff2 = dict(K=4 * D, bias=P.ff2.b, **drop.at(2))
    ff2.update(dict(self_resid=True) if P.self_resid else dict(resid=v(L.x1)))
    if form == "fused":
        head = dict(att=L.att, W=P.proj.w, h1=L.h1, gamma=P.ln1.gamma, beta=P.ln1.beta, mean=L.mean1, rstd=L.rstd1, **proj)
        kw = dict(x=L.x1, W1=P.ff1.w, a_out=L.a, W2=P.ff2.w, h_out=L.h2, gamma=P.ln2.gamma, beta=P.ln2.beta, y_out=L.x2, mean=L.mean2,
                  rstd=L.rstd2, ff1=ff1, ff2=ff2, proj=head, row_groups=row_groups)
        if not launch:
            return kw
        o.ffn_ln_fwd(**kw)
        return L.x2
    o.gemm_nt(v(L.att), P.proj.w, L.h1, c_remap=rows.c_remap, **proj)
    o.layernorm_fwd(v(L.h1), P.ln1.gamma, P.ln1.beta, v(L.x1), L.mean1, L.rstd1, D=D, **rows.ln)
    o.gemm_nt(v(L.x1), P.ff1.w, L.a, c_remap=rows.c_remap, **ff1)
    o.gemm_nt(v(L.a), P.ff2.w, L.h2, c_remap=rows.c_remap, **ff2)
    o.layernorm_fwd(v(L.h2), P.ln2.gamma, P.ln2.beta, v(L.x2), L.mean2, L.rstd2, D=D, **rows.ln)
    return L.x2


def _lead_mask(P, t, drop):
    if P.mask_mode == 2:
        return dict(mask_mode=2, **drop.at(2))
    return dict(mask_mode=1, dx_masked=t.dhm, **drop.at(2)) if drop.p > 0 else {}


def no_partials(norm, parts):
    return None


def ffn_bwd_parts(L, row_groups=None):
    M = L.h1.shape[0]
    return o.gemm_nt_ln_parts(M if row_groups is None else M // row_groups[1] * row_groups[0])


def ffn_bwd_kw(P, L, t, drop, partials_buf, row_groups=None):
    dff = t.dhm if (drop.p > 0 and not P.self_resid) else t.dh
    ln1 = dict(dx_masked=t.dh1m, mask_mode=1, **drop.at(0)) if drop.p > 0 else {}
    return dict(dff=dff, W2t=P.ff2.t, dpre_out=t.dpre, gate=L.a, W1t=P.ff1.t, dx_out=t.dh1, x=L.h1, gamma=P.ln1.gamma, mean=L.mean1,
                rstd=L.rstd1, dgamma=P.ln1.dgamma, dbeta=P.ln1.dbeta, alpha=1.0 / (1.0 - drop.p) if drop.p > 0 else 1.0,
                resid=None if P.self_resid else t.dh, partials=partials_buf, row_groups=row_groups, **ln1)


def row_block_bwd(P, L, t, dy, rows, drop, form, partials, dy_done=False, row_groups=None, tail=None, launch=True):
    D, v = P.proj.w.shape[0], rows.view
    if form == "tail":
        o.row_tail_bwd(v(dy), v(L.h2), v(L.h1), v(L.a), L.mean1, L.rstd1, L.mean2, L.rstd2, P.ln1.gamma, P.ln2.gamma, P.ff2.t, P.ff1.t,
                       P.proj.t, t.dh, t.dhm, t.dx1, t.dh1m, t.dpre, v(t.dh1), v(t.datt), P.ln1.dgamma, P.ln1.dbeta, P.ln2.dgamma,
                       P.ln2.dbeta, dropout_p=drop.p, dropout_seed_ptr=drop.seed_ptr, site0=drop.site0, **tail)
        return t.dhm, t.dh1m
    M = L.h1.shape[0]
    lead = None
    if not dy_done and form == "fused" and P.mask_mode == 1:
        lead = dict(dy=dy, x=L.h2, gamma=P.ln2.gamma, mean=L.mean2, rstd=L.rstd2, dx=t.dh, dgamma=P.ln2.dgamma, dbeta=P.ln2.dbeta,
                    partials=partials(P.ln2, o.gemm_nt_ln_parts(M)), **_lead_mask(P, t, drop))
    elif not dy_done:
        mask = _lead_mask(P, t, drop)
        if P.mask_mode == 2:
            mask["dropout_site"] = drop.site0 + 2
        o.layernorm_bwd(v(L.h2), P.ln2.gamma, L.mean2, L.rstd2, v(dy), t.dh, P.ln2.dgamma, P.ln2.dbeta, D=D,
                        partials=partials(P.ln2, o.layernorm_bwd_parts(M, D)), **rows.ln, **mask)
    dff = t.dhm if (drop.p > 0 and not P.self_resid) else t.dh
    resid_ff = None if P.self_resid else t.dh
    inv_keep = 1.0 / (1.0 - drop.p) if drop.p > 0 else 1.0
    ln1 = dict(dx_masked=t.dh1m, mask_mode=1, **drop.at(0)) if drop.p > 0 else {}
    if form == "fused":
        buf = partials(P.ln1, ffn_bwd_parts(L, row_groups))
        if launch:
            o.ffn_ln_bwd(lead=lead, **ffn_bwd_kw(P, L, t, drop, buf, row_groups))
        elif lead is not None:
            raise ValueError("row_block_bwd(launch=False) needs dy_done: the block that ran elsewhere has no leading LayerNorm backward")
    else:
        o.gemm_nt(dff, P.ff2.t, t.dpre, N=4 * D, K=D, gate=v(L.a), alpha=inv_keep)
        if form == "ln_fused":
            o.gemm_nt_ln_bwd(t.dpre, P.ff1.t, t.dh1, L.h1, P.ln1.gamma, L.mean1, L.rstd1, P.ln1.dgamma, P.ln1.dbeta, N=D, K=4 * D,
                             resid=resid_ff, partials=partials(P.ln1, o.gemm_nt_ln_parts(M)), **ln1)
        else:
            o.gemm_nt(t.dpre, P.ff1.t, t.dx1, N=D, K=4 * D, resid=resid_ff)
            o.layernorm_bwd(v(L.h1), P.ln1.gamma, L.mean1, L.rstd1, t.dx1, v(t.dh1), P.ln1.dgamma, P.ln1.dbeta, D=D,
                            partials=partials(P.ln1, o.layernorm_bwd_parts(M, D)), **rows.ln, **ln1)
    dproj = t.dh1m if drop.p > 0 else v(t.dh1)
    o.gemm_nt(dproj, P.proj.t, t.datt, N=D, K=D, c_remap=rows.c_remap)
    return dff, dproj


def layer_wgrads(P, L, t, x_in, dff, dproj, rows):
    D, v = P.proj.w.shape[0], rows.view
    return [o.wgrad_problem(dff, v(L.a), P.ff2.dw, P.ff2.db, N=D, K=4 * D),
            o.wgrad_problem(t.dpre, v(L.x1), P.ff1.dw, P.ff1.db, N=4 * D, K=D),
            o.wgrad_problem(dproj, v(L.att), P.proj.dw, P.proj.db, N=D, K=D),
            o.wgrad_problem(t.dqkv, x_in, P.kqv.dw, P.kqv.db, N=3 * D, K=D)]


def row_tail_selfcheck(store, B=64, S=2):
    store.tail_checked = True
    cfg, dev, adt = store.cfg, store.device, store.act_dtype
    D, F = cfg.e_model, 4 * cfg.e_model
    if not (o.can_row_tail(B, D) and store.tail_fused and cfg.e_layers >= 1):
        return True
    f32 = dict(dtype=torch.float32, device=dev)
    P = store.layer("encoder", cfg.e_layers - 1)
    scratch = lambda n: n._replace(dgamma=torch.zeros(D, **f32), dbeta=torch.zeros(D, **f32))
    P = P._replace(ln1=scratch(P.ln1), ln2=scratch(P.ln2))

    def rnd(n, width, site):
        a = torch.zeros(n, width, **f32)
        o.randn(a, seed=0x7A11, site=site)
        t = torch.zeros(n, width, dtype=adt, device=dev)
        o.cast_to_act(a, t)
        return t

    z = lambda n, w: torch.zeros(n, w, dtype=adt, device=dev)
    att, xin = rnd(B * S, D, 1), rnd(B * S, D, 2)
    status = torch.zeros(2, dtype=torch.int32, device=dev)
    sync = torch.zeros(8, dtype=torch.int32, device=dev)
    rows = position0_rows(B, S)

    def fbufs():
        L = _Layer()
        L.att, L.h1, L.x1, L.a, L.h2, L.x2 = att, z(B * S, D), z(B * S, D), z(B * S, F), z(B * S, D), z(B * S, D)
        L.mean1, L.rstd1, L.mean2, L.rstd2 = (torch.zeros(B * S, **f32) for _ in range(4))
        return L

    u, f = fbufs(), fbufs()
    tail = dict(stat_stride=S, phys_stride=S, status=status[0:1])
    row_block_fwd(P, u, xin, rows, NO_DROPOUT, "launches")
    row_block_fwd(P, f, xin, rows, NO_DROPOUT, "tail", tail=dict(tail, sync=sync[0:3]))
    dy = rnd(B * S, D, 3)

    def bbufs():
        t = _Layer()
        t.dh, t.dhm, t.dx1, t.dh1m, t.dpre, t.dh1, t.datt = z(B, D), z(B, D), z(B, D), z(B, D), z(B, F), z(B * S, D), z(B * S, D)
        return t

    ub, fb = bbufs(), bbufs()
    row_block_bwd(P, u, ub, dy, rows, NO_DROPOUT, "launches", no_partials)
    row_block_bwd(P, u, fb, dy, rows, NO_DROPOUT, "tail", no_partials, tail=dict(tail, sync=sync[4:7]))
    torch.cuda.current_stream().synchronize()
    want_f, want_b = o.row_tail_barriers(D)
    sy, stv = sync.cpu().tolist(), status.cpu().tolist()
    why = []
    if stv[0]:
        why.append(f"status flags {stv[0]:#x}")
    if sy[0] != want_f or sy[4] != want_b:
        why.append(f"barrier counters {sy[0]} / {sy[4]} instead of {want_f} / {want_b}")
    ulp = 2.0 ** -7 if adt == torch.bfloat16 else 2.0 ** -10
    host = lambda t: t.float().cpu().numpy()
    for k in ("h1", "x1", "a", "h2", "x2"):
        a, b = host(rows.view(getattr(f, k))), host(rows.view(getattr(u, k)))
        if not np.all(np.abs(a - b) <= 4 * ulp * np.maximum(np.abs(b), 1.0)):
            why.append(f"forward {k}: max difference {np.abs(a - b).max():.3g}")
    for k in ("dh", "dpre", "dx1", "dh1", "datt"):
        a, b = host(getattr(fb, k)), host(getattr(ub, k))
        if not np.abs(a - b).max() <= 4 * ulp * max(float(np.abs(b).max()), 1e-6) + 1e-6:
            why.append(f"backward {k}: max difference {np.abs(a - b).max():.3g} (scale {np.abs(b).max():.3g})")
    if why:
        store.tail_fused = False
        warnings.warn("the one-launch position-0 tail failed its start-up check on this device (" + "; ".join(why) +
                      "): using the five-launch form", RuntimeWarning)
    return not why


Forms = namedtuple("Forms", "tails riders shadows fuse_bce bce_dgrad skip_row0 cls_fold ffn_e ffn_d ln_bwd_e ln_bwd_d sched dec_tail gnorm ema")


def check_schedule(kl_warmup_steps=0, kl_cycle_steps=0, kl_free_bits=0.0, lr_warmup_steps=0):
    for name, val in (("kl_warmup_steps", kl_warmup_steps), ("kl_cycle_steps", kl_cycle_steps), ("lr_warmup_steps", lr_warmup_steps)):
        if int(val) != val or val < 0:
            raise ValueError(f"{name} must be a non-negative integer, not {val!r}")
    if not kl_free_bits >= 0:
        raise ValueError(f"kl_free_bits must be >= 0 nats per sample, not {kl_free_bits!r}")
    if kl_cycle_steps > 0 and kl_warmup_steps == 0:
        raise ValueError("kl_cycle_steps restarts the KL warm-up: it needs kl_warmup_steps > 0")
    if kl_cycle_steps > 0 and kl_warmup_steps > kl_cycle_steps:
        raise ValueError(f"kl_warmup_steps ({kl_warmup_steps}) must not exceed kl_cycle_steps ({kl_cycle_steps})")


def check_clip(clip_global_norm=0.0):
    if not (0 <= clip_global_norm < float("inf")):
        raise ValueError(f"clip_global_norm must be 0 (off) or a positive finite norm, not {clip_global_norm!r}")


def clip_scale(norm, max_norm):
    c = np.float32(max_norm) / (np.float32(norm) + np.float32(1e-8))
    return c if c < np.float32(1) else np.float32(1)


def check_ema(ema_decay=0.0):
    if not (0 <= ema_decay < 1):
        raise ValueError(f"ema_decay must be 0 (off) or lie in (0, 1), not {ema_decay!r}")


def ema_decay_at(t, decay):
    tf = np.float32(t)
    d = (np.float32(1) + tf) / (np.float32(10) + tf)
    return min(np.float32(decay), d)


def ema_update(e, w_new, d):
    d = np.float32(d)
    omd = np.float32(1) - d
    a = d * np.asarray(e, np.float32)
    b = omd * np.asarray(w_new, np.float32)
    return a + b


def schedule_values(t, kl_weight=1.0, kl_warmup_steps=0, kl_cycle_steps=0, lr_warmup_steps=0):
    f_lr = min(1.0, t / lr_warmup_steps) if lr_warmup_steps > 0 else 1.0
    u = (t - 1) % kl_cycle_steps + 1 if kl_cycle_steps > 0 else t
    ramp = min(1.0, u / kl_warmup_steps) if kl_warmup_steps > 0 else 1.0
    return float(np.float32(float(np.float32(kl_weight)) * ramp)), f_lr


class StepPlan:

    def __init__(self, store, B, T, lr=3e-4, clip_gradient=1.0, kl_weight=1.0, label_smoothing=0.0,
                 negative_label_downscaling=False, global_batch=None, gscale=None, want_probs=False, seed=0,
                 internal_eps=False, optimizer_params=None, sample_offset=0, site_base=0,
                 kl_warmup_steps=0, kl_cycle_steps=0, kl_free_bits=0.0, lr_warmup_steps=0, clip_global_norm=0.0, ema_decay=0.0):
        cfg = store.cfg
        self.store, self.cfg, self.B, self.T = store, cfg, B, T
        self.dev, self.adt = store.device, store.act_dtype
        self.lr, self.clip, self.kl_weight = lr, clip_gradient, kl_weight
        check_schedule(kl_warmup_steps, kl_cycle_steps, kl_free_bits, lr_warmup_steps)
        self.schedule = dict(kl_warmup_steps=int(kl_warmup_steps), kl_cycle_steps=int(kl_cycle_steps), kl_free_bits=float(kl_free_bits),
                             lr_warmup_steps=int(lr_warmup_steps))
        self.scheduled = any(self.schedule.values())
        check_clip(clip_global_norm)
        self.clip_global_norm = float(clip_global_norm)
        self.grad_parts = store.grad_parts() if self.clip_global_norm > 0 else None
        check_ema(ema_decay)
        self.ema_decay = float(ema_decay)
        if self.ema_decay > 0:
            store.enable_ema()
        self.ls, self.nld = label_smoothing, negative_label_downscaling
        self.global_batch = global_batch or B
        self.sample_offset, self.site_base = int(sample_offset), int(site_base)
        if (self.sample_offset * cfg.latent_dim) % 2:
            raise ValueError("sample_offset * latent_dim must be even (eps is drawn in Box-Muller pairs)")
        self.gscale = gscale if gscale is not None else (1024.0 if self.adt == torch.float16 else 1.0)
        self.gscale_enc = 1.0
        self.want_probs, self.internal_eps = want_probs, internal_eps
        self.opt = dict(beta1=0.9, beta2=0.999, eps=1e-8, wd=0.0)
        if optimizer_params:
            for k_src, k_dst in (("beta1", "beta1"), ("beta2", "beta2"), ("epsilon", "eps"), ("wd", "wd")):
                if k_src in optimizer_params:
                    self.opt[k_dst] = float(optimizer_params[k_src])
        dev, adt = self.dev, self.adt
        De, Dd, Z = cfg.e_model, cfg.d_model, cfg.latent_dim
        Se, Sd = T, T + 1
        self.Me, self.Md = B * Se, B * Sd
        f32 = dict(dtype=torch.float32, device=dev)

        def act(rows, width):
            return torch.zeros(rows, roundup(width, 8), dtype=adt, device=dev)

        self.ride = (cfg.kind != "token" and cfg.d_layers >= 1 and cfg.e_layers >= 1 and Dd in (128, 256) and
                     o.can_ride(B * T, 3 * Dd, Dd, T) and o.can_ride(B * T, Dd, 3 * Dd, T))
        self.shadows_on_tail = True
        self.dec_tail = True
        self.n_cu = torch.cuda.get_device_properties(self.dev).multi_processor_count if self.dev.type == "cuda" else 0
        self.forms = self._resolve_forms()
        if cfg.kind == "token":
            seg = [("tokens", B * T * 4), ("labels", B * T * 4)]
        else:
            self.ld_roll = roundup(cfg.in_dim + (cfg.num_classes if self.forms.cls_fold else 0), 8)
            seg = [("roll", B * T * self.ld_roll), ("labels", B * T * cfg.out_dim)]
        seg += [("seq_lens", B * 4), ("classes", B * 4)]
        self.in_layout, off = {}, 0
        for name, nbytes in seg:
            self.in_layout[name] = (off, nbytes)
            off = roundup(off + nbytes, 16)
        self.own_inbuf = torch.zeros(off, dtype=torch.uint8, device=dev)
        self.bind_inputs(self.own_inbuf)
        self.eps = torch.zeros(B, Z, **f32)
        self.rng_state = store.rng_state(seed)
        self._outers = []

        self.pos_e = torch.from_numpy(positional_table(De, Se)).to(dev)
        self.pos_d = torch.from_numpy(positional_table(Dd, Sd)).to(dev)
        self.keymask_e = torch.zeros(B, Se, dtype=torch.uint8, device=dev)
        self.keymask_d = torch.zeros(B, Sd, dtype=torch.uint8, device=dev)

        def layers(n, M, D, H, S):
            out = []
            for _ in range(n):
                L = _Layer()
                L.qkv, L.att, L.h1, L.x1 = act(M, 3 * D), act(M, D), act(M, D), act(M, D)
                L.a, L.h2, L.x2 = act(M, 4 * D), act(M, D), act(M, D)
                L.lse = torch.zeros(2, B, H, S, **f32)
                L.mean1, L.rstd1 = torch.zeros(M, **f32), torch.zeros(M, **f32)
                L.mean2, L.rstd2 = torch.zeros(M, **f32), torch.zeros(M, **f32)
                out.append(L)
            return out

        self.x0_e = act(self.Me, De)
        self.enc = layers(cfg.e_layers, self.Me, De, cfg.e_heads, Se)
        self.x0_d = act(self.Md, Dd)
        self.dec = layers(cfg.d_layers, self.Md, Dd, cfg.d_heads, Sd)
        self.mu, self.sigma, self.z = torch.zeros(B, Z, **f32), torch.zeros(B, Z, **f32), torch.zeros(B, Z, **f32)
        self.kl, self.total = torch.zeros(B, **f32), torch.zeros(B, **f32)
        nb4 = (B + 3) // 4 * 4
        self._recon_buf = torch.zeros(nb4 + 8 + 24 + 64, **f32)
        self.recon = self._recon_buf[:B]
        self.sync_words = self._recon_buf[nb4: nb4 + 8].view(torch.int32)
        self.ride_queues = self._recon_buf[nb4 + 32:].view(torch.int32)
        self.metric_acc = store.metric_acc
        self.track_token_metrics = False
        self.logits = None if self.forms.fuse_bce else act(B * T, cfg.out_dim)
        self.dlogits = act(B * T, cfg.out_dim)
        if cfg.kind == "token":
            self.probs = torch.zeros(B * T, cfg.out_dim, **f32) if want_probs else None
        else:
            self.probs = act(B * T, cfg.out_dim) if want_probs else None
        self.npos = torch.zeros(B, dtype=torch.int32, device=dev)

        def bwd_bufs(M, D, H, S):
            t = _Layer()
            t.dx_a, t.dx_b = act(M, D), act(M, D)
            t.dh, t.dhm = act(M, D), act(M, D)
            t.dh1, t.dh1m = act(M, D), act(M, D)
            t.dpre, t.dx1 = act(M, 4 * D), act(M, D)
            t.datt, t.dqkv = act(M, D), act(M, 3 * D)
            t.delta = torch.zeros(B, H, S, **f32)
            return t

        self.be_l = [bwd_bufs(self.Me, De, cfg.e_heads, Se) for _ in range(cfg.e_layers)]
        self.bd_l = [bwd_bufs(self.Md, Dd, cfg.d_heads, Sd) for _ in range(cfg.d_layers)]
        self._wgrads = []
        self.wgrad_scratch = store.wgrad_scratch()
        self._ln_part, self._psums = {}, []
        for side, n_l, M, D in (("encoder", cfg.e_layers, self.Me, De), ("decoder", cfg.d_layers, self.Md, Dd)):
            rows = max(o.layernorm_bwd_parts(M, D), o.gemm_nt_ln_parts(M))
            for i in range(n_l):
                for ln in ("ln1", "ln2" if side == "encoder" else "ln3"):
                    self._ln_part[f"{side}.layer{i}.{ln}"] = torch.zeros(rows, 2 * D, **f32)
        self.lat_scratch = torch.zeros(B * (Dd + 2 * Z), **f32)
        self.d_dec_out = act(self.Md, Dd)
        self.d_enc_out = act(self.Me, De)
        c = _Layer()
        c.dh, c.dhm, c.dx1, c.dh1m = act(B, De), act(B, De), act(B, De), act(B, De)
        c.dpre = act(B, 4 * De)
        self.sp_dh1 = c.dh1 = act(self.Me, De)
        self.sp_datt = c.datt = act(self.Me, De)
        c.dqkv, c.delta = self.be_l[-1].dqkv, self.be_l[-1].delta
        self.top = c
        self.graph = None
        self.graph_late = None
        self.graph_opt = None
        self._tick_adam = False
        self._infer = False
        self._tail_used = dict(fwd=False, bwd=False)
        if o.can_row_tail(B, De) and store.tail_fused and not store.tail_checked:
            row_tail_selfcheck(store)

    @property
    def e_p(self):
        return 0.0 if self._infer else self.cfg.e_dropout

    @property
    def d_p(self):
        return 0.0 if self._infer else self.cfg.d_dropout

    def _resolve_forms(self, with_grad=False):
        cfg, st, B, T = self.cfg, self.store, self.B, self.T
        De, Dd = cfg.e_model, cfg.d_model
        roll = cfg.kind == "pianoroll"
        tails = bool(o.can_row_tail(B, De) and st.tail_fused)
        riders = bool(self.ride and tails)
        shadows = "own" if not st.shadows_deferred else ("tail" if self.shadows_on_tail and riders else "begin")
        fuse_bce = roll and o.can_fuse_bce(cfg.out_dim, T, self.nld) and o.bce_fusion_pays(cfg.out_dim)
        ffn_d, ln_bwd_d = o.ffn_fusion_pays(Dd, 4 * Dd), o.ln_bwd_fusion_pays(Dd)
        bce_dgrad = fuse_bce and ln_bwd_d
        skip_row0 = cfg.d_layers > 0 and T % 64 == 0 and ffn_d
        return Forms(
            tails=tails, riders=riders, shadows=shadows, fuse_bce=fuse_bce,
            bce_dgrad=bce_dgrad,
            skip_row0=skip_row0,
            dec_tail=bool(with_grad and not self._infer and self.dec_tail and bce_dgrad and ffn_d and skip_row0 and
                          o.dec_tail_pays(Dd, 4 * Dd, cfg.out_dim, T, B * T // 64, self.n_cu)),
            cls_fold=(roll and cfg.in_dim % 8 == 0 and roundup(cfg.in_dim + cfg.num_classes, 256) == roundup(cfg.in_dim, 256) and
                      st.offsets["encoder.class2hid.weight"] == st.offsets["encoder.embedding.weight"] + cfg.in_dim * De),
            ffn_e=o.ffn_fusion_pays(De, 4 * De), ffn_d=ffn_d, ln_bwd_e=o.ln_bwd_fusion_pays(De), ln_bwd_d=ln_bwd_d,
            sched=self.scheduled,
            gnorm=self.clip_global_norm > 0,
            ema=self.ema_decay > 0)

    def _guard(self):
        fwd, bwd = o.row_tail_barriers(self.cfg.e_model)
        exp = []
        if self._tail_used["fwd"]:
            exp.append((self.sync_words[0:1], fwd))
        if self._tail_used["bwd"]:
            exp.append((self.sync_words[4:5], bwd))
        g = dict(status=self.store.step_status, expect=exp)
        if self.global_batch == self.B:
            g["finite"] = (self.recon, self.kl)
        return g

    def bind_inputs(self, buf):
        cfg, B, T = self.cfg, self.B, self.T
        need = max(a + n for a, n in self.in_layout.values())
        if not (buf.dtype == torch.uint8 and buf.is_contiguous() and buf.is_cuda and buf.data_ptr() % 16 == 0 and buf.numel() >= need):
            raise ValueError("bind_inputs: need a contiguous, 16-byte aligned device uint8 blob of pack_batch()'s size")
        self.inbuf = buf

        def inview(name, dtype, *shape):
            a, n = self.in_layout[name]
            return buf[a: a + n].view(dtype).view(*shape)

        if cfg.kind == "token":
            self.tokens = inview("tokens", torch.int32, B, T)
            self.labels = inview("labels", torch.int32, B, T)
        else:
            self.roll_cls = inview("roll", torch.uint8, B * T, self.ld_roll)
            self.roll = self.roll_cls[:, : roundup(cfg.in_dim, 8)]
            self.labels = inview("labels", torch.uint8, B * T, cfg.out_dim)
        self.seq_lens = inview("seq_lens", torch.int32, B)
        self.classes = inview("classes", torch.int32, B)

    def load_batch(self, x, seq_lens, classes, labels, eps=None):
        def dev(a, dtype):
            t = torch.as_tensor(np.asarray(a)) if not torch.is_tensor(a) else a
            return t.to(device=self.dev, dtype=dtype, non_blocking=True)

        cfg, B, T = self.cfg, self.B, self.T
        if cfg.kind == "token":
            self.tokens.copy_(dev(x, torch.int32).view(B, T))
            self.labels.copy_(dev(labels, torch.int32).view(B, T))
        else:
            self.roll[:, : cfg.in_dim].copy_(dev(x, torch.uint8).view(B * T, cfg.in_dim))
            self.labels.copy_(dev(labels, torch.uint8).view(B * T, cfg.out_dim))
        self.seq_lens.copy_(dev(seq_lens, torch.int32))
        self.classes.copy_(dev(classes, torch.int32))
        if self.forms.cls_fold:
            w = self.ld_roll - cfg.in_dim
            onehot = (self.classes.view(B, 1).to(torch.int64) == torch.arange(w, device=self.dev).view(1, w)).to(torch.uint8)
            self.roll_cls.view(B, T, -1)[:, :, cfg.in_dim:].copy_(onehot.view(B, 1, w).expand(B, T, w))
        if eps is not None:
            self.eps.copy_(dev(eps, torch.float32))

    def pack_into(self, blob, x, seq_lens, classes, labels):
        cfg, B, T = self.cfg, self.B, self.T
        assert blob.dtype == torch.uint8 and not blob.is_cuda and blob.numel() >= self.inbuf.numel()
        raw = blob.numpy()

        def seg(name, dtype, *shape):
            a, n = self.in_layout[name]
            return raw[a: a + n].view(dtype).reshape(*shape)

        def as_np(a):
            return a.cpu().numpy() if torch.is_tensor(a) else np.asarray(a)

        if cfg.kind == "token":
            np.copyto(seg("tokens", np.int32, B, T), as_np(x).reshape(B, T), casting="unsafe")
            np.copyto(seg("labels", np.int32, B, T), as_np(labels).reshape(B, T), casting="unsafe")
        else:
            ldp = self.ld_roll
            roll = seg("roll", np.uint8, B * T, ldp)
            np.copyto(roll[:, : cfg.in_dim], as_np(x).reshape(B * T, cfg.in_dim), casting="unsafe")
            if self.forms.cls_fold:
                w = ldp - cfg.in_dim
                roll.reshape(B, T, ldp)[:, :, cfg.in_dim:] = (as_np(classes).reshape(B, 1, 1).astype(np.int64) ==
                                                              np.arange(w).reshape(1, 1, w)).astype(np.uint8)
            elif ldp != cfg.in_dim:
                roll[:, cfg.in_dim:] = 0
            np.copyto(seg("labels", np.uint8, B * T, cfg.out_dim), as_np(labels).reshape(B * T, cfg.out_dim), casting="unsafe")
        np.copyto(seg("seq_lens", np.int32, B), as_np(seq_lens).reshape(B), casting="unsafe")
        np.copyto(seg("classes", np.int32, B), as_np(classes).reshape(B), casting="unsafe")
        return blob

    def pack_batch(self, x, seq_lens, classes, labels):
        return self.pack_into(torch.zeros(self.inbuf.numel(), dtype=torch.uint8), x, seq_lens, classes, labels)

    def load_packed(self, blob):
        self.inbuf.copy_(blob, non_blocking=True)

    def _drop(self, p, site):
        return dict(dropout_p=p, dropout_site=site, dropout_seed_ptr=self.rng_state) if p > 0 else {}

    def _dropout(self, p, site0):
        return Dropout(p, self.rng_state if p > 0 else None, site0)

    def _site_e(self, i):
        return self.site_base + 3 * i

    def _site_d(self, i):
        return self.site_base + 3 * (self.cfg.e_layers + i)

    def _late_shadows(self):
        st = self.store
        return dict(w=st.w, wt16=st.wt16, desc=st.t_desc_late, prefix=st.t_prefix_late, n_mat=st.t_n_late, tiles=st.t_tiles_late)

    def _top_encoder_layer_fwd(self, i, L, x_in):
        cfg, st, B, S, F = self.cfg, self.store, self.B, self.T, self.forms
        D, H = cfg.e_model, cfg.e_heads
        P = st.layer("encoder", i)
        o.attn_qkv_fwd(x_in, P.kqv.w, P.kqv.b, L.qkv, self.keymask_e, L.lse, L.att, B, S, H, D // H, 0, D, 2 * D, q_limit=1)
        self._tail_used["fwd"] = F.tails
        tail = None
        if F.tails:
            tail = dict(sync=self.sync_words[0:3], stat_stride=S, phys_stride=S, status=st.step_status[0:1], queue=self.ride_queues[0:1])
            if F.riders:
                Pd, Dd, Sd = st.layer("decoder", 0), cfg.d_model, S + 1
                tail["rider"] = dict(A=self.x0_d, B=Pd.kqv.w, C_out=self.dec[0].qkv, M=B * S, N=3 * Dd, K=Dd, bias=Pd.kqv.b,
                                     a_remap=(S, Sd, 1), c_remap=(S, Sd, 1))
                if F.shadows == "tail":
                    tail["shadows"] = self._late_shadows()
        return row_block_fwd(P, L, x_in, position0_rows(B, S), self._dropout(self.e_p, self._site_e(i)),
                             "tail" if F.tails else "launches", tail=tail)

    def _layer_fwd(self, side, i, L, x_in, keymask, D, H, S, p, site0):
        F = self.forms
        dh = D // H
        if side == "encoder" and i == self.cfg.e_layers - 1:
            return self._top_encoder_layer_fwd(i, L, x_in)
        P = self.store.layer(side, i)
        causal = side == "decoder" and self.cfg.d_causal
        if side == "decoder" and i == 0 and F.riders:
            (o.attn_causal_fwd if causal else o.attn_fwd)(L.qkv, keymask, L.lse, L.att, self.B, S, H, dh, 0, D, 2 * D)
        elif causal:
            o.gemm_nt(x_in, P.kqv.w, L.qkv, N=3 * D, K=D, bias=P.kqv.b)
            o.attn_causal_fwd(L.qkv, keymask, L.lse, L.att, self.B, S, H, dh, 0, D, 2 * D)
        else:
            o.attn_qkv_fwd(x_in, P.kqv.w, P.kqv.b, L.qkv, keymask, L.lse, L.att, self.B, S, H, dh, 0, D, 2 * D)
        fused = F.ffn_e if side == "encoder" else F.ffn_d
        if F.dec_tail and side == "decoder" and i == self.cfg.d_layers - 1:
            return L.x2
        return row_block_fwd(P, L, x_in, ALL_ROWS, self._dropout(p, site0), "fused" if fused else "launches",
                             row_groups=self._row0_groups(side, i))

    def _row0_groups(self, side, i):
        if side == "decoder" and i == self.cfg.d_layers - 1 and self.forms.skip_row0:
            return (self.T, self.T + 1, 1)
        return None

    def forward(self, inference=False, upto=None, with_grad=False):
        if with_grad and (inference or upto):
            raise ValueError("forward(with_grad=True) is the forward pass of a training step")
        if upto not in (None, "latent") or (upto and not inference):
            raise ValueError("forward(upto=...) takes 'latent', in inference mode only")
        cfg, st, B, T = self.cfg, self.store, self.B, self.T
        self._infer = bool(inference)
        F = self.forms = self._resolve_forms(with_grad)
        self._tail_used = dict(fwd=False, bwd=False)
        De, Dd = cfg.e_model, cfg.d_model
        Se, Sd = T, T + 1
        sq_e, sq_d = math.sqrt(float(De)), math.sqrt(float(Dd))
        self._wgrads, self._psums, self._outers = [], [], []
        need_rng = self.e_p > 0 or self.d_p > 0 or self.internal_eps
        rng = st.rng_state_inference() if self._infer else self.rng_state
        tick = self._tick_adam and not self._infer
        begin = dict(rng_state=rng if need_rng else None,
                     adam_state=st.step_state if tick else None, lr=self.lr, beta1=self.opt["beta1"],
                     beta2=self.opt["beta2"], eps_out=self.eps if self.internal_eps else None,
                     eps_index0=self.sample_offset * cfg.latent_dim, lens=self.seq_lens,
                     mask_e=self.keymask_e if cfg.kind != "token" else None, add_e=0, mask_d=self.keymask_d, add_d=1,
                     zero_a=self._recon_buf, zero_b=st.g if tick else None)
        if F.shadows == "begin":
            begin["shadows"] = self._late_shadows()
        if F.sched and tick:
            begin["schedule"] = dict(block=st.sched, kl_weight=self.kl_weight, **self.schedule)
        ride = cfg.kind != "token"
        if not ride:
            o.step_begin(**begin)
        if cfg.kind == "token":
            o.embed_fwd(self.tokens, st.p("encoder.embedding.weight"), self.pos_e, self.x0_e.view(B, Se, -1), 0, sq_e,
                        classes=self.classes, cls_table=st.p("encoder.class2hid.weight"), keymask=self.keymask_e)
        else:
            o.gemm_nt_pair(dict(A=self.roll, B=st.t("encoder.embedding.weight"), C_out=self.x0_e, N=De, alpha=sq_e,
                                grpadd=st.p("encoder.class2hid.weight"), grp_index=self.classes, rowadd=self.pos_e, rowadd_period=T),
                           dict(A=self.roll, B=st.t("decoder.embedding.weight"), C_out=self.x0_d, M=B * T, N=Dd, alpha=sq_d,
                                rowadd=self.pos_d[1:], rowadd_period=T, c_remap=(T, Sd, 1)),
                           begin=begin if ride else None)
        x = self.x0_e
        for i, L in enumerate(self.enc):
            x = self._layer_fwd("encoder", i, L, x, self.keymask_e, De, cfg.e_heads, Se, self.e_p, self._site_e(i))
        self.enc_out = x
        lat = (x.view(B, Se, -1), st.p("encoder.latent_proj.weight"), st.p("encoder.latent_proj.bias"), self.eps,
               st.p("decoder.latent2hid.weight"), st.p("decoder.latent2hid.bias"), self.classes,
               st.p("decoder.class2hid.weight"), self.pos_d, sq_d, self.mu, self.sigma, self.z, self.kl,
               self.x0_d.view(B, Sd, -1))
        proj0 = None
        if F.riders:
            Pd = st.layer("decoder", 0)
            proj0 = (Pd.kqv.w, Pd.kqv.b, self.dec[0].qkv.view(B, Sd, -1))
        o.latent_fwd(*lat, proj=proj0)
        if upto == "latent":
            return
        if cfg.kind == "token":
            o.embed_fwd(self.tokens, st.p("decoder.embedding.weight"), self.pos_d, self.x0_d.view(B, Sd, -1), 1, sq_d)
        x = self.x0_d
        site_d = self._site_d(0)
        for i, L in enumerate(self.dec):
            x = self._layer_fwd("decoder", i, L, x, self.keymask_d, Dd, cfg.d_heads, Sd, self.d_p, site_d + 3 * i)
        self.dec_out = x
        if not F.fuse_bce:
            o.gemm_nt(x, st.h("decoder.output_layer.weight"), self.logits, M=B * T, K=Dd, bias=st.p("decoder.output_layer.bias"),
                      a_remap=(T, Sd, 1))

    def losses(self, with_grad=True, combine=True):
        cfg, B, T, F = self.cfg, self.B, self.T, self.forms
        dl = self.dlogits if with_grad else None
        if cfg.kind == "token":
            o.softmax_ce(self.logits, self.labels, self.recon, B, T, cfg.out_dim, probs=self.probs, dlogits=dl,
                         gscale=self.gscale, pre_zeroed=True,
                         tok_parts=self.store.tok_parts if self.track_token_metrics else None)
        elif F.fuse_bce:
            dgrad = None
            if F.dec_tail and not with_grad:
                raise RuntimeError("forward(with_grad=True) left the last decoder layer to losses(with_grad=True)")
            if with_grad and F.bce_dgrad:
                last, Dd, Sd = cfg.d_layers - 1, cfg.d_model, T + 1
                dgrad = dict(A=self.dlogits, B=self.store.t("decoder.output_layer.weight"), dX_out=self.bd_l[last].dh, M=B * T, N=Dd,
                             K=self.dlogits.shape[1], c_remap=(T, Sd, 1),
                             **self._out_ln_bwd("decoder", last, self.dec[last], cfg.d_dropout, self._site_d(0) + 3 * last,
                                                self.bd_l[last], B * T))
            loss = dict(A=self.dec_out, B=self.store.h("decoder.output_layer.weight"), labels=self.labels, loss=self.recon, T=T,
                        dlogits=dl, probs=self.probs, label_smoothing=self.ls, downweight=self.nld, gscale=self.gscale, M=B * T,
                        K=cfg.d_model, bias=self.store.p("decoder.output_layer.bias"), a_remap=(T, T + 1, 1))
            if F.dec_tail:
                L, t, P = self.dec[last], self.bd_l[last], self.store.layer("decoder", last)
                drop, groups = self._dropout(self.d_p, self._site_d(0) + 3 * last), self._row0_groups("decoder", last)
                x_in = self.dec[last - 1].x2 if last > 0 else self.x0_d
                o.dec_tail_step(row_block_fwd(P, L, x_in, ALL_ROWS, drop, "fused", row_groups=groups, launch=False), loss, dgrad,
                                ffn_bwd_kw(P, L, t, drop, self._ln_partials_buf(P.ln1, ffn_bwd_parts(L, groups)), groups))
            else:
                o.gemm_sigmoid_bce(dgrad=dgrad, **loss)
        else:
            o.sigmoid_bce(self.logits, self.labels, self.recon, B, T, cfg.out_dim, label_smoothing=self.ls,
                          downweight=self.nld, npos=self.npos, probs=self.probs, dlogits=dl, gscale=self.gscale,
                          pre_zeroed=True)
        if combine:
            o.loss_combine(self.recon, self.kl, self.kl_weight, self.total, self.metric_acc, guard=self._guard())

    LN_PARTIALS_MIN = 32

    def _ln_partials_buf(self, norm, parts):
        return self._ln_part[norm.site] if parts >= self.LN_PARTIALS_MIN else None

    def _ln_partials(self, norm, parts):
        buf, dg, db = self._ln_partials_buf(norm, parts), norm.dgamma, norm.dbeta
        if buf is None:
            return None
        D = dg.numel()
        if db.data_ptr() == dg.data_ptr() + 4 * D:
            self._psums.append(o.partial_sum_job(buf, parts, dg, length=2 * D))
        else:
            self._psums += [o.partial_sum_job(buf, parts, dg, length=D), o.partial_sum_job(buf, parts, db, col_off=D, length=D)]
        return buf

    def _flush_grads(self):
        o.gemm_wgrad_batch(self._wgrads, scratch=self.wgrad_scratch, sums=self._psums, outers=self._outers)
        self.last_wgrad_launch = (self._wgrads, self._psums)
        self._wgrads, self._psums, self._outers = [], [], []

    def _out_ln_bwd(self, side, i, L, p, site0, t, M):
        P = self.store.layer(side, i)
        return dict(x=L.h2, gamma=P.ln2.gamma, mean=L.mean2, rstd=L.rstd2, dgamma=P.ln2.dgamma, dbeta=P.ln2.dbeta,
                    partials=self._ln_partials(P.ln2, o.gemm_nt_ln_parts(M)), **_lead_mask(P, t, self._dropout(p, site0)))

    def _layer_bwd(self, side, i, L, x_in, dy, dx_in, keymask, D, H, S, p, site0, t, dy_done=False, next_ln=None, ride=False):
        F, P = self.forms, self.store.layer(side, i)
        ffn, ln = (F.ffn_e, F.ln_bwd_e) if side == "encoder" else (F.ffn_d, F.ln_bwd_d)
        in_loss = F.dec_tail and side == "decoder" and i == self.cfg.d_layers - 1
        dff, dproj = row_block_bwd(P, L, t, dy, ALL_ROWS, self._dropout(p, site0), "fused" if ffn else ("ln_fused" if ln else "launches"),
                                   self._ln_partials, dy_done=dy_done, row_groups=self._row0_groups(side, i), launch=not in_loss)
        if side == "decoder" and self.cfg.d_causal:
            o.attn_causal_bwd(L.qkv, keymask, L.lse, t.datt, t.dqkv, t.delta, self.B, S, H, D // H, 0, D, 2 * D)
        else:
            o.attn_bwd(L.qkv, keymask, L.lse, t.datt, t.dqkv, t.delta, self.B, S, H, D // H, 0, D, 2 * D)
        handed = None
        if next_ln is not None:
            kw, t_below = next_ln
            o.gemm_nt_ln_bwd(t.dqkv, P.kqv.t, t_below.dh, N=D, K=3 * D, resid=t.dh1, **kw)
        elif ride:
            T_ = self.T
            handed = (dict(A=t.dqkv, B=P.kqv.t, C_out=dx_in, M=self.B * T_, N=D, K=3 * D, resid=t.dh1, resid_phys=True,
                           a_remap=(T_, T_ + 1, 1), c_remap=(T_, T_ + 1, 1)),
                      (t.dqkv.view(self.B, S, -1), P.kqv.t, t.dh1.view(self.B, S, -1)))
        else:
            o.gemm_nt(t.dqkv, P.kqv.t, dx_in, N=D, K=3 * D, resid=t.dh1)
        self._wgrads += layer_wgrads(P, L, t, x_in, dff, dproj, ALL_ROWS)
        return handed

    def _top_encoder_layer_bwd(self, i, L, x_in, dx_in, next_ln=None, rider=None):
        cfg, st, B, S, F = self.cfg, self.store, self.B, self.T, self.forms
        D, H = cfg.e_model, cfg.e_heads
        P, c, rows = st.layer("encoder", i), self.top, position0_rows(B, S)
        self._tail_used["bwd"] = F.tails
        tail = None
        if F.tails:
            tail = dict(sync=self.sync_words[4:7], stat_stride=S, phys_stride=S, status=st.step_status[0:1], rider=rider,
                        queue=self.ride_queues[32:33])
        dff, dproj = row_block_bwd(P, L, c, self.d_enc_out, rows, self._dropout(cfg.e_dropout, self._site_e(i)),
                                   "tail" if F.tails else "launches", no_partials, tail=tail)
        o.attn_bwd(L.qkv, self.keymask_e, L.lse, c.datt, c.dqkv, c.delta, B, S, H, D // H, 0, D, 2 * D, q_limit=1)
        if next_ln is not None:
            kw, t_below = next_ln
            o.gemm_nt_ln_bwd(c.dqkv, P.kqv.t, t_below.dh, N=D, K=3 * D, resid=c.dh1, **kw)
        else:
            o.gemm_nt(c.dqkv, P.kqv.t, dx_in, N=D, K=3 * D, resid=c.dh1)
        self._wgrads += layer_wgrads(P, L, c, x_in, dff, dproj, rows)

    def backward(self):
        self.backward_early(flush=False)
        self.backward_late()

    def grad_cut(self):
        cfg, st = self.cfg, self.store
        if cfg.e_layers < 2:
            return 0
        return st.offsets[f"encoder.layer{cfg.e_layers - 1}.att.W_k.weight"]

    def _below(self, side, i, fuse):
        if not (fuse and i > 0):
            return None
        if side == "encoder":
            layers, bufs, p, site0, M = self.enc, self.be_l, self.cfg.e_dropout, self._site_e(i - 1), self.Me
        else:
            layers, bufs, p, site0, M = self.dec, self.bd_l, self.cfg.d_dropout, self._site_d(i - 1), self.Md
        return self._out_ln_bwd(side, i - 1, layers[i - 1], p, site0, bufs[i - 1], M), bufs[i - 1]

    def backward_early(self, flush):
        cfg, st, B, T, F = self.cfg, self.store, self.B, self.T, self.forms
        De, Dd = cfg.e_model, cfg.d_model
        Se, Sd = T, T + 1
        sq_d = math.sqrt(float(Dd))
        ldv = self.dlogits.shape[1]
        site_d = self._site_d(0)
        last = cfg.d_layers - 1
        if F.bce_dgrad:
            pass
        elif F.ln_bwd_d:
            o.gemm_nt_ln_bwd(self.dlogits, st.t("decoder.output_layer.weight"), self.bd_l[last].dh, M=B * T, N=Dd, K=ldv,
                             c_remap=(T, Sd, 1),
                             **self._out_ln_bwd("decoder", last, self.dec[last], cfg.d_dropout, site_d + 3 * last, self.bd_l[last], B * T))
        else:
            o.gemm_nt(self.dlogits, st.t("decoder.output_layer.weight"), self.d_dec_out, M=B * T, N=Dd, K=ldv, c_remap=(T, Sd, 1))
        self._wgrads.append(o.wgrad_problem(self.dlogits, self.dec_out, st.grad("decoder.output_layer.weight"),
                                            st.grad("decoder.output_layer.bias"), M=B * T, N=cfg.out_dim, K=Dd, b_remap=(T, Sd, 1)))
        dy, pingpong, handed = self.d_dec_out, (self.bd_l[0].dx_a, self.bd_l[0].dx_b), None
        for n, i in enumerate(reversed(range(cfg.d_layers))):
            x_in = self.dec[i - 1].x2 if i > 0 else self.x0_d
            handed = self._layer_bwd("decoder", i, self.dec[i], x_in, dy, pingpong[n % 2], self.keymask_d, Dd, cfg.d_heads, Sd,
                                     cfg.d_dropout, site_d + 3 * i, self.bd_l[i], dy_done=F.ln_bwd_d,
                                     next_ln=self._below("decoder", i, F.ln_bwd_d), ride=F.riders and i == 0)
            dy = pingpong[n % 2]
        d_x0_d = dy
        rider, dx0 = handed or (None, None)
        if cfg.kind == "token":
            o.embed_bwd(self.tokens, st.grad("decoder.embedding.weight"), d_x0_d.view(B, Sd, -1), 1, sq_d)
        else:
            self._wgrads.append(o.wgrad_problem(self.roll, d_x0_d, st.grad("decoder.embedding.weight"), M=B * T, N=cfg.out_dim,
                                                K=Dd, scale=sq_d, b_remap=(T, Sd, 1)))
        d_enc = self.d_enc_out
        o.latent_bwd_vec(st.p("encoder.latent_proj.weight"), self.eps, st.p("decoder.latent2hid.weight"), self.classes, self.mu,
                         self.sigma, d_x0_d.view(B, Sd, -1), sq_d, self.kl_weight, self.gscale_enc,
                         st.grad("decoder.class2hid.weight"), d_enc.view(B, Se, -1), self.lat_scratch,
                         enc_scale=self.gscale_enc / self.gscale, proj=dx0, sched=(st.sched, self.kl) if F.sched else None)
        self._outers += o.latent_outer_jobs(self.lat_scratch, self.enc_out.view(B, Se, -1), self.z,
                                            st.grad("encoder.latent_proj.weight"), st.grad("encoder.latent_proj.bias"),
                                            st.grad("decoder.latent2hid.weight"), st.grad("decoder.latent2hid.bias"))
        top = cfg.e_layers - 1
        x_in = self.enc[top - 1].x2 if top > 0 else self.x0_e
        self._top_encoder_layer_bwd(top, self.enc[top], x_in, self.be_l[0].dx_a, next_ln=self._below("encoder", top, F.ln_bwd_e),
                                    rider=rider)
        if flush and cfg.e_layers >= 2:
            self._flush_grads()

    def backward_late(self):
        cfg, st, B, T, F = self.cfg, self.store, self.B, self.T, self.forms
        De, Se = cfg.e_model, T
        sq_e = math.sqrt(float(De))
        dy, pingpong = self.be_l[0].dx_a, (self.be_l[0].dx_b, self.be_l[0].dx_a)
        for n, i in enumerate(reversed(range(cfg.e_layers - 1))):
            x_in = self.enc[i - 1].x2 if i > 0 else self.x0_e
            self._layer_bwd("encoder", i, self.enc[i], x_in, dy, pingpong[n % 2], self.keymask_e, De, cfg.e_heads, Se, cfg.e_dropout,
                            self._site_e(i), self.be_l[i], dy_done=F.ln_bwd_e, next_ln=self._below("encoder", i, F.ln_bwd_e))
            dy = pingpong[n % 2]
        d_x0_e = dy
        if cfg.kind == "token":
            o.embed_bwd(self.tokens, st.grad("encoder.embedding.weight"), d_x0_e.view(B, Se, -1), 0, sq_e,
                        classes=self.classes, dcls=st.grad("encoder.class2hid.weight"))
        else:
            self._wgrads.append(o.wgrad_problem(self.roll_cls, d_x0_e, st.grad("encoder.embedding.weight"), M=B * T,
                                                N=cfg.in_dim + (cfg.num_classes if F.cls_fold else 0), K=De, scale=sq_e))
            if not F.cls_fold:
                o.group_colsum(d_x0_e.view(B, Se, -1), T, De, 0, self.classes, st.grad("encoder.class2hid.weight"), sq_e)
        self._flush_grads()

    def optimizer(self):
        st = self.store
        deferred = self.forms.shadows != "own"
        sched = st.sched if self.forms.sched else None
        clip = self.clip if self.clip is not None else -1.0
        guard = self._guard()
        mt = dict(recon=self.recon, kl=self.kl, kl_weight=self.kl_weight, total=self.total, metric=self.metric_acc, **guard)
        emb = (lambda base: dict(base=base, specs=st.emb_specs, wt16=st.wt16)) if deferred else (lambda base: None)
        gn = ((lambda a: dict(gnorm=dict(parts=self.grad_parts, max_norm=self.clip_global_norm, gstat=st.gstat if a == 0 else None)))
              if self.forms.gnorm else (lambda a: {}))
        av = (lambda a, b: dict(ema=dict(buf=st.ema[a:b], decay=self.ema_decay))) if self.forms.ema else (lambda a, b: {})
        if self.gscale == self.gscale_enc:
            r = 1.0 / (self.global_batch * self.gscale)
            if self.forms.gnorm:
                o.grad_sumsq(st.g, 0, r, r, self.grad_parts)
            o.adam_flat(st.w, st.g, st.m, st.v, st.w16, st.step_state, lr=self.lr,
                        rescale=r, clip=clip, advance_step=False, metrics=mt, emb=emb(0),
                        sched=sched, **gn(0), **av(0, st.n), **self.opt)
        else:
            cut = st.offsets["decoder.latent2hid.weight"]
            rng = [(0, cut, self.gscale_enc, False), (cut, st.n, self.gscale, False)]
            if self.forms.gnorm:
                o.grad_sumsq(st.g, cut, 1.0 / (self.global_batch * self.gscale_enc), 1.0 / (self.global_batch * self.gscale), self.grad_parts)
            for a, b, gs, adv in rng:
                o.adam_flat(st.w[a:b], st.g[a:b], st.m[a:b], st.v[a:b], st.w16[a:b], st.step_state, lr=self.lr,
                            rescale=1.0 / (self.global_batch * gs), clip=clip, advance_step=adv,
                            metrics=mt if a == 0 else (guard or None), emb=emb(a), sched=sched if a == 0 else None, **gn(a),
                            **av(a, b), **self.opt)
        if not deferred:
            o.transpose_shadows(st.w, st.wt16, st.t_desc, st.t_prefix, len(st.t_specs), st.t_tiles)

# ... 76 lines not shown
```

### musicstyletransfer_amd/ops.py

```python
import ctypes as C
import math

import torch

from . import _lib
from ._lib import LnArgs, LnBwdIn, PartialSum, OuterJob, StepBeginArgs, StepMetrics, ACT_NONE, ACT_RELU, MST_BF16, MST_F16, GemmArgs, WgradArgs, call

_DT = {torch.bfloat16: MST_BF16, torch.float16: MST_F16}


def dt(x):
    try:
        return _DT[x if isinstance(x, torch.dtype) else x.dtype]
    except KeyError:
        raise TypeError(f"activation dtype must be bfloat16 or float16, got {x}") from None


def ptr(t):
    if t is None:
        return None
    assert t.is_cuda, "mst ops need device tensors (there is no CPU fallback)"
    if t.device.index != torch.cuda.current_device():
        raise RuntimeError(f"tensor on cuda:{t.device.index} but the current device is cuda:{torch.cuda.current_device()}: "
                           "call torch.cuda.set_device() for this rank's GPU first")
# ... 268 lines not shown


def ffn_ln_bwd(dff, W2t, dpre_out, gate, W1t, dx_out, x, gamma, mean, rstd, dgamma, dbeta, alpha=1.0, dx_masked=None, mask_mode=0,
               partials=None, lead=None, row_groups=None, **kw):
    g1, g2, l = _ffn_ln_bwd_args(dff, W2t, dpre_out, gate, W1t, dx_out, x, gamma, mean, rstd, dgamma, dbeta, alpha, dx_masked, mask_mode,
                                 partials, row_groups, **kw)
    if lead is None:
        call("mst_ffn_ln_bwd", C.byref(g1), C.byref(g2), C.byref(l), stream())
        return
    q = LnBwdIn()
    q.dy, q.ld_dy = ptr(lead["dy"]), ld(lead["dy"])
    q.x, q.ld_x = ptr(lead["x"]), ld(lead["x"])
    q.gamma, q.mean, q.rstd = ptr(lead["gamma"]), ptr(lead["mean"]), ptr(lead["rstd"])
    q.dx, q.ld_dx = ptr(lead["dx"]), ld(lead["dx"])
    dxm = lead.get("dx_masked")
    q.dx_masked, q.ld_dxm = ptr(dxm), (ld(dxm) if dxm is not None else 0)
    q.dgamma, q.dbeta, q.partials = ptr(lead.get("dgamma")), ptr(lead.get("dbeta")), ptr(lead.get("partials"))
    q.mask_mode = 1 if dxm is not None else 0
    q.dropout_p, q.dropout_seed = lead.get("dropout_p", 0.0), lead.get("dropout_seed", 0)
    q.dropout_seed_ptr, q.dropout_site = ptr(lead.get("dropout_seed_ptr")), lead.get("dropout_site", 0)
    if lead.get("partials") is not None:
        assert lead["partials"].shape[0] >= gemm_nt_ln_parts(g1.M) and lead["partials"].shape[1] == 2 * g2.N
    call("mst_ffn_ln_bwd_lead", C.byref(q), C.byref(g1), C.byref(g2), C.byref(l), stream())


def gemm_nt_ln_bwd(A, B, dX_out, x, gamma, mean, rstd, dgamma, dbeta, dx_masked=None, mask_mode=0, partials=None, **kw):
    g, l = _gemm_ln_bwd_args(A, B, dX_out, x, gamma, mean, rstd, dgamma, dbeta, dx_masked, mask_mode, partials, **kw)
    call("mst_gemm_nt_ln", C.byref(g), C.byref(l), stream())


def _gemm_ln_bwd_args(A, B, dX_out, x, gamma, mean, rstd, dgamma, dbeta, dx_masked=None, mask_mode=0, partials=None, **kw):
    g = _gemm_args(A, B, dX_out, **kw)
    l = LnArgs()
    l.mode, l.gamma = 2, ptr(gamma)
    l.mean, l.rstd = ptr(mean), ptr(rstd)
    l.x, l.ld_x = ptr(x), ld(x)
    l.dgamma, l.dbeta = ptr(dgamma), ptr(dbeta)
    l.out, l.ld_out = ptr(dx_masked), (ld(dx_masked) if dx_masked is not None else 0)
    l.mask_mode = mask_mode
    l.partials = ptr(partials)
    if partials is not None:
        assert partials.shape[0] >= gemm_nt_ln_parts(g.M) and partials.shape[1] == 2 * g.N and partials.is_contiguous()
    return g, l


def gemm_nt_ln_parts(M):
    return int(_lib.load().mst_gemm_nt_ln_parts(M))


def layernorm_bwd_parts(M, D):
    return int(_lib.load().mst_layernorm_bwd_parts(M, D))


PARTIAL_SUM_MAX_JOBS = 20


def partial_sum_job(src, n_parts, dst, scale=1.0, col_off=0, length=None):
    j = PartialSum()
    length = dst.numel() if length is None else length
    assert src.dtype == dst.dtype and src.element_size() == 4 and src.shape[0] >= n_parts
    j.src = src.data_ptr() + 4 * col_off
    j.n_parts, j.stride, j.len = n_parts, src.stride(0), length
    j.dst, j.scale = ptr(dst), scale
    return j


def partial_sums(jobs):
    for i in range(0, len(jobs), PARTIAL_SUM_MAX_JOBS):
        chunk = jobs[i:i + PARTIAL_SUM_MAX_JOBS]
        call("mst_partial_sums", (PartialSum * len(chunk))(*chunk), len(chunk), stream())


def wgrad_problem(A, B, dW, db=None, M=None, N=None, K=None, scale=1.0, a_remap=(0, 0, 0), b_remap=(0, 0, 0)):
    w = WgradArgs()
    w.a_u8 = 1 if A.dtype == torch.uint8 else 0
    w.dtype = dt(B if w.a_u8 else A)
    w.M = A.shape[0] if M is None else M
    w.N = dW.shape[0] if N is None else N
    w.K = dW.shape[1] if K is None else K
    w.A, w.lda = ptr(A), ld(A)
    w.B, w.ldb = ptr(B), ld(B)
    w.dW, w.ldw = ptr(dW), ld(dW)
    w.db = ptr(db)
    w.scale = scale
    w.a_rows_per_group, w.a_group_stride, w.a_group_offset = a_remap
    w.b_rows_per_group, w.b_group_stride, w.b_group_offset = b_remap
    return w


WGRAD_MAX_PROBLEMS = 16
OUTER_MAX_JOBS = 2


def outer_job(L, R, out, obias=None):
    q = OuterJob()
    assert L.dtype == torch.float32 and L.is_contiguous() and out.dtype == torch.float32 and out.is_contiguous() and R.stride(1) == 1
    q.L, q.R, q.r_stride = ptr(L), ptr(R), R.stride(0)
    q.r_dtype = 2 if R.dtype == torch.float32 else dt(R)
    q.B, q.J, q.I = L.shape[0], L.shape[1], R.shape[1]
    assert out.numel() == q.J * q.I and R.shape[0] == q.B and (obias is None or obias.numel() == q.J)
    q.out, q.obias = ptr(out), ptr(obias)
    return q


def outer_jobs(jobs):
    for i in range(0, len(jobs), OUTER_MAX_JOBS):
        chunk = jobs[i:i + OUTER_MAX_JOBS]
        call("mst_outer_jobs", (OuterJob * len(chunk))(*chunk), len(chunk), stream())


def gemm_wgrad_batch(problems, scratch=None, sums=None, outers=None):
    sums, outers = list(sums or []), list(outers or [])
    for i in range(0, len(problems), WGRAD_MAX_PROBLEMS):
        chunk = problems[i:i + WGRAD_MAX_PROBLEMS]
        take, tko = [], []
        if i + WGRAD_MAX_PROBLEMS >= len(problems):
            take, sums = sums[:PARTIAL_SUM_MAX_JOBS], sums[PARTIAL_SUM_MAX_JOBS:]
            tko, outers = outers[:OUTER_MAX_JOBS], outers[OUTER_MAX_JOBS:]
        call("mst_gemm_wgrad_batch_flush", (WgradArgs * len(chunk))(*chunk), len(chunk), ptr(scratch),
             (scratch.numel() * scratch.element_size() if scratch is not None else 0),
             (PartialSum * len(take))(*take) if take else None, len(take),
             (OuterJob * len(tko))(*tko) if tko else None, len(tko), stream())
    if sums:
        partial_sums(sums)
    if outers:
        outer_jobs(outers)


def gemm_wgrad_plan(problems, scratch_bytes=0):
    plan = (C.c_int64 * (4 + WGRAD_MAX_PROBLEMS))()
    call("mst_gemm_wgrad_plan", (WgradArgs * len(problems))(*problems), len(problems), scratch_bytes, plan)
    return dict(form=plan[0], narrow=plan[1], items=plan[2], two_pass=plan[3], splits=list(plan[4:4 + len(problems)]))


def gemm_wgrad(A, B, dW, db=None, **kw):
    gemm_wgrad_batch([wgrad_problem(A, B, dW, db, **kw)])


def attn_fwd(qkv, keymask, lse, out, B, S, H, dh, k_off, q_off, v_off, q_limit=0):
    call("mst_attn_keysoftmax_fwd", dt(qkv), B, S, H, dh, ptr(qkv), ld(qkv), k_off, q_off, v_off, ptr(keymask),
         ptr(lse), ptr(out), ld(out), q_limit, stream())


def attn_qkv_fwd(x, W, bias, qkv, keymask, lse, out, B, S, H, dh, k_off, q_off, v_off, q_limit=0):
    call("mst_attn_qkv_fwd", dt(qkv), B, S, H, dh, ptr(x), ld(x), ptr(W), ld(W), ptr(bias), ptr(qkv), ld(qkv), k_off, q_off, v_off,
         ptr(keymask), ptr(lse), ptr(out), ld(out), q_limit, stream())


def attn_bwd(qkv, keymask, lse, dout, dqkv, delta, B, S, H, dh, k_off, q_off, v_off, q_limit=0):
    call("mst_attn_keysoftmax_bwd", dt(qkv), B, S, H, dh, ptr(qkv), ld(qkv), k_off, q_off, v_off, ptr(keymask),
         ptr(lse), ptr(dout), ld(dout), ptr(dqkv), ld(dqkv), ptr(delta), q_limit, stream())


ATTN_FWD_PATHS = ("resident-3", "resident-2", "chunked", "fused", "stream")
ATTN_BWD_PATHS = ("resident", "stream+chunked-dq", "stream")


def attn_fwd_form(dtype, B, S, H, dh, k_off, q_off, v_off, ld_qkv, ld_out, q_limit=0, fused=False, ld_x=0, ld_w=0):
    form = (C.c_int64 * 8)()
    call("mst_attn_fwd_form", dt(dtype), B, S, H, dh, ld_qkv, k_off, q_off, v_off, ld_out, q_limit, 1 if fused else 0, ld_x, ld_w, form)
    return dict(path=ATTN_FWD_PATHS[form[0]], waves=form[1], lds=form[2], lone=form[3], grid_stats=form[4], grid_out=form[5])


def attn_bwd_form(dtype, B, S, H, dh, k_off, q_off, v_off, ld_qkv, ld_dout, ld_dqkv, q_limit=0):
    form = (C.c_int64 * 8)()
    call("mst_attn_bwd_form", dt(dtype), B, S, H, dh, ld_qkv, k_off, q_off, v_off, ld_dout, ld_dqkv, q_limit, form)
    return dict(path=ATTN_BWD_PATHS[form[0]], waves=form[1], lds=form[2], sparse=form[3], lone=form[4], dq_chunks=form[5],
                dq_waves=form[6])


def attn_causal_fwd(qkv, keymask, lse, out, B, S, H, dh, k_off, q_off, v_off):
    call("mst_attn_causal_fwd", dt(qkv), B, S, H, dh, ptr(qkv), ld(qkv), k_off, q_off, v_off, ptr(keymask), ptr(lse), ptr(out),
         ld(out), stream())


def attn_causal_bwd(qkv, keymask, lse, dout, dqkv, delta, B, S, H, dh, k_off, q_off, v_off):
    call("mst_attn_causal_bwd", dt(qkv), B, S, H, dh, ptr(qkv), ld(qkv), k_off, q_off, v_off, ptr(keymask), ptr(lse), ptr(dout),
         ld(dout), ptr(dqkv), ld(dqkv), ptr(delta), stream())


def attn_decode(cache3, n_keys, H, dh, k_off, q_off, v_off, out, mode=0):
    B, t_max = cache3.shape[0], cache3.shape[1]
    assert cache3.stride(2) == 1 and cache3.stride(0) == t_max * cache3.stride(1)
    call("mst_attn_decode", dt(cache3), B, H, dh, n_keys, t_max, ptr(cache3), cache3.stride(1), k_off, q_off, v_off, mode, ptr(out),
         ld(out), stream())


def beam_step(probs, scores_in, scores_out, seqs_in, seqs_out, hyp_src, word, i, K, eos, pad, active=None):
    N, V = probs.shape[0], probs.shape[1]
    call("mst_beam_step", N // K, K, V, i, seqs_in.shape[1], ptr(probs), probs.stride(0), ptr(scores_in), ptr(scores_out), ptr(seqs_in),
         ptr(seqs_out), ptr(hyp_src), ptr(word), ptr(active), eos, pad, stream())


def sample_step(probs, seqs, scores, word, i, seed, eos, pad, active=None):
    call("mst_sample_step", probs.shape[0], probs.shape[1], i, seqs.shape[1], ptr(probs), probs.stride(0), ptr(seqs), ptr(scores), ptr(word),
         ptr(active), seed, eos, pad, stream())


FRAME_MODES = {"draw": 0, "threshold": 1}


def frame_step(logits, P, i, seed_ptr, frames, roll, scores, tau=1.0, mode="draw", thr=0.5, probs_out=None):
    N, L = roll.shape[0], roll.shape[1]
    assert roll.is_contiguous() and (probs_out is None or (probs_out.is_contiguous() and tuple(probs_out.shape) == (N, L, P)))
    call("mst_frame_step", dt(logits), N, P, i, L, ptr(logits), ld(logits), tau, FRAME_MODES[mode], thr, ptr(seed_ptr), ptr(frames), ld(frames),
         ptr(roll), roll.stride(1), ptr(scores), ptr(probs_out), stream())


def token_step(logits, V, i, seed_ptr, seqs, scores, word, eos, pad, tau=1.0, top_k=0, top_p=1.0, active=None, kept_out=None):
    assert seqs.is_contiguous()
    call("mst_token_step", dt(logits), seqs.shape[0], V, i, seqs.shape[1], ptr(logits), ld(logits), tau, top_k, top_p, ptr(seed_ptr), ptr(seqs),
         ptr(scores), ptr(word), ptr(active), ptr(kept_out), eos, pad, stream())


def beam_gather(cache_in, cache_out, src, n_rows, skip_cols=None):
    N, t_max, width = cache_in.shape
    es = cache_in.element_size()
    if skip_cols is None:
        call("mst_beam_gather", ptr(cache_in), ptr(cache_out), ptr(src), N, n_rows, width * es, t_max, stream())
    else:
        call("mst_beam_gather_cols", ptr(cache_in), ptr(cache_out), ptr(src), N, n_rows, width * es, t_max, skip_cols[0] * es,
             skip_cols[1] * es, stream())


def layernorm_fwd(x, gamma, beta, y, mean, rstd, D=None, eps=1e-5, M=None, row_id_stride=1):
    M = x.shape[0] if M is None else M
    D = x.shape[1] if D is None else D
    call("mst_layernorm_fwd", dt(x), M, D, ptr(x), ld(x), ptr(gamma), ptr(beta), eps, ptr(y), ld(y), ptr(mean),
         ptr(rstd), row_id_stride, stream())


def layernorm_bwd(x, gamma, mean, rstd, dy, dx, dgamma, dbeta, D=None, dx_masked=None, mask_mode=0, dropout_p=0.0,
                  dropout_seed=0, dropout_site=0, dropout_seed_ptr=None, M=None, row_id_stride=1, partials=None):
    M = x.shape[0] if M is None else M
    D = x.shape[1] if D is None else D
    if partials is not None:
        assert partials.shape[0] >= layernorm_bwd_parts(M, D) and partials.shape[1] == 2 * D and partials.is_contiguous()
    call("mst_layernorm_bwd", dt(x), M, D, ptr(x), ld(x), ptr(gamma), ptr(mean), ptr(rstd), ptr(dy), ld(dy), ptr(dx),
         ld(dx), ptr(dx_masked), (ld(dx_masked) if dx_masked is not None else 0), ptr(dgamma), ptr(dbeta), mask_mode,
         dropout_p, dropout_seed, dropout_site, ptr(dropout_seed_ptr), row_id_stride, ptr(partials), stream())


def embed_fwd(tokens, table, pos, out3, s_off, alpha, classes=None, cls_table=None, keymask=None):
    B, T = tokens.shape
    D = table.shape[1]
    call("mst_embed_fwd", dt(out3), B, T, D, ptr(tokens), ptr(table), table.stride(0), ptr(classes), ptr(cls_table),
         (cls_table.stride(0) if cls_table is not None else 0), ptr(pos), pos.stride(0), alpha, ptr(out3),
         out3.stride(1), out3.shape[1], s_off, ptr(keymask), stream())


def embed_bwd(tokens, dtable, dX3, s_off, alpha, classes=None, dcls=None):
    B, T = tokens.shape
    D = dtable.shape[1]
    call("mst_embed_bwd", dt(dX3), B, T, D, ptr(tokens), ptr(dtable), dtable.stride(0), ptr(classes), ptr(dcls),
         (dcls.stride(0) if dcls is not None else 0), alpha, ptr(dX3), dX3.stride(1), dX3.shape[1], s_off, stream())


def group_colsum(X3, T, D, s_off, idx, dst, alpha):
    B = X3.shape[0]
    call("mst_group_colsum", dt(X3), B, T, D, ptr(X3), X3.stride(1), X3.shape[1], s_off, ptr(idx), ptr(dst),
         dst.stride(0), alpha, stream())


def mask_from_lengths(lens, add, keymask):
    B, S = keymask.shape
    call("mst_mask_from_lengths", B, S, ptr(lens), add, ptr(keymask), stream())


def latent_fwd(enc_out3, Wl, bl, eps, Wh, bh, classes, cls_d, pos_d, alpha_d, mu, sigma, z, kl, dec_in3, proj=None):
    B = enc_out3.shape[0]
    De, Z, Dd = Wl.shape[1], Wh.shape[1], Wh.shape[0]
    args = (dt(enc_out3), B, De, Z, Dd, ptr(enc_out3), enc_out3.stride(0), ptr(Wl), ptr(bl), ptr(eps),
            ptr(Wh), ptr(bh), ptr(classes), ptr(cls_d), cls_d.stride(0), ptr(pos_d), alpha_d, ptr(mu), ptr(sigma), ptr(z),
            ptr(kl), ptr(dec_in3), dec_in3.stride(0))
    if proj is None:
        call("mst_latent_fwd", *args, stream())
    else:
        Wq, bq, qkv3 = proj
        call("mst_latent_fwd_proj", *args, ptr(Wq), ld(Wq), ptr(bq), ptr(qkv3), qkv3.stride(0), Wq.shape[0], stream())


def latent_form(De, Z, Dd, nq=0, Wl=0, part=None):
    form = (C.c_int64 * 8)(*([-1] * 8))
    addr = Wl.data_ptr() if isinstance(Wl, torch.Tensor) else Wl
    rc = _lib.load().mst_latent_form(De, Z, Dd, nq, addr, form)
    names = ("fwd_pre", "loader_l", "loader_h", "proj_vec", "fwd_lds", "bwd_pre", "dh0", "bwd_lds")
    if part == "fwd" and form[0] >= 0:
        return dict(zip(names[:5], form[:5]))
    _lib.check(rc, "mst_latent_form")
    return dict(zip(names[5:], form[5:8])) if part == "bwd" else dict(zip(names, form))


LATENT_ROWS_SITE = 0x7FFE0000
INTERP = {"lerp": 0, "slerp": 1}


def latent_rows(zsrc, ssrc, a, b, w, ca, cb, cw, Wh, bh, cls_d, pos_d, alpha_d, z_out, dec_in, mode="lerp", tau=0.0, seed=0, seed_ptr=None,
                row0=0, site=LATENT_ROWS_SITE):
    N, (Dd, Z) = z_out.shape[0], Wh.shape
    M = zsrc.shape[0] if zsrc is not None else 0
    assert z_out.is_contiguous() and z_out.shape[1] == Z and (zsrc is None or (zsrc.is_contiguous() and zsrc.shape[1] == Z))
    assert ssrc is None or (zsrc is not None and ssrc.shape == zsrc.shape and ssrc.is_contiguous())
    for t in (a, b, w, ca, cb, cw):
        assert t is None or (t.numel() == N and t.is_contiguous())
    call("mst_latent_rows", dt(dec_in), N, M, Z, Dd, ptr(zsrc), ptr(ssrc), ptr(a), ptr(b), ptr(w), INTERP[mode], tau,
         seed & 0xFFFFFFFFFFFFFFFF, ptr(seed_ptr), site, row0, ptr(Wh), ptr(bh), ptr(ca), ptr(cb), ptr(cw), ptr(cls_d), cls_d.stride(0),
         cls_d.shape[0], ptr(pos_d), alpha_d, ptr(z_out), ptr(dec_in), ld(dec_in), stream())


def latent_bwd_vec(Wl, eps, Wh, classes, mu, sigma, d_dec_in3, alpha_d, kl_weight, gscale, dcls_d, d_enc_out3, scratch, enc_scale=1.0,
                   proj=None, sched=None):
    B, De, Z, Dd = d_dec_in3.shape[0], Wl.shape[1], Wh.shape[1], Wh.shape[0]
    if sched is not None:
        assert sched[0].dtype == sched[1].dtype == torch.float32 and sched[0].numel() >= 4 and sched[1].numel() == B
    weight = (kl_weight,) if sched is None else (ptr(sched[0]), ptr(sched[1]))
    suffix = "" if sched is None else "_sched"
    if proj is not None:
        dq3, Wt, r3 = proj
        call("mst_latent_bwd_vec_proj" + suffix, dt(dq3), B, De, Z, Dd, ptr(Wl), ptr(eps), ptr(Wh), ptr(classes), ptr(mu), ptr(sigma),
             ptr(dq3), dq3.stride(0), ptr(Wt), ld(Wt), 3 * Dd, ptr(r3), (r3.stride(0) if r3 is not None else 0), alpha_d, *weight,
             gscale, enc_scale, ptr(dcls_d), dcls_d.stride(0), ptr(d_enc_out3), d_enc_out3.stride(0), ptr(scratch), stream())
# ... 267 lines not shown
```

Before: 26.20 million frames/s.

## Fuse attention output-projection dgrad GEMM into resident attention backward kernel

Adds a prologue to the resident attention backward kernel that computes each head's dOut slice as dproj·W_projᵀ directly into LDS with MFMA, so the separate gemm_nt launch and the round trip of datt through global memory are no longer needed. The engine enables this per side when a form rule allows it (dense path, head size ≤32, one wave per 32-row block, LDS budget). Each workgroup now recomputes a head-slice GEMM over the full model width. This adds LDS pressure and may lower occupancy or lengthen the kernel's critical path.

```diff
diff --git a/include/mst_hip.h b/include/mst_hip.h
--- a/include/mst_hip.h
+++ b/include/mst_hip.h
@@ -183,6 +183,10 @@
                             void* dqkv, int64_t ld_dqkv, float* delta,
                             int64_t q_limit ,
                             mst_stream_t stream);
+int mst_attn_proj_bwd(int dtype, int64_t B, int64_t S, int64_t H, int64_t dh, const void* qkv, int64_t ld_qkv, int64_t k_off,
+                      int64_t q_off, int64_t v_off, const uint8_t* keymask, const float* lse, const void* dproj, int64_t ld_dproj,
+                      const void* wt, int64_t ld_wt, void* dout_out, int64_t ld_dout, void* dqkv, int64_t ld_dqkv, float* delta,
+                      mst_stream_t stream);
 
 int mst_attn_fwd_form(int dtype, int64_t B, int64_t S, int64_t H, int64_t dh, int64_t ld_qkv, int64_t k_off, int64_t q_off,
                       int64_t v_off, int64_t ld_out, int64_t q_limit, int fused, int64_t ld_x, int64_t ld_w, int64_t* form);
diff --git a/musicstyletransfer_amd/csrc/attention.hip b/musicstyletransfer_amd/csrc/attention.hip
--- a/musicstyletransfer_amd/csrc/attention.hip
+++ b/musicstyletransfer_amd/csrc/attention.hip
@@ -1063,8 +1063,127 @@
   }
 }
 
-template <typename T, int DH, bool SPARSE>
+constexpr int DOP_KC = 64;
+constexpr int DOP_LDS = DOP_KC + 8;
+__device__ __forceinline__ void wave_lds_fence() {
+  __builtin_amdgcn_fence(__ATOMIC_RELEASE, "wavefront");
+  __builtin_amdgcn_wave_barrier();
+  __builtin_amdgcn_fence(__ATOMIC_ACQUIRE, "wavefront");
+}
+template <typename T, int DH>
+__device__ __forceinline__ void dout_prologue(const AttnArgs& a, unsigned char* smem, T* bufA, T* bufB, const T* __restrict__ Qg, int64_t b,
+                                              int64_t hd, int NB, bool lone) {
+  constexpr int LD = LdsLd<DH>::V, TN = DH / 16, TMX = DH <= 16 ? 3 : 2, CPR = DH / 8;
+  typedef typename Act<T>::vec8 vec8;
+  const int tid = threadIdx.x, lane = tid & 63, wave = tid >> 6, nthr = blockDim.x, NW = nthr >> 6;
+  const int64_t S = a.S;
+  const int SP = NB * 32, D = (int)a.Dm, LDW = D + 8, nch = D / DOP_KC;
+  T* const sX = reinterpret_cast<T*>(smem);
+  T* const sW = sX + SP * DOP_LDS;
+  const T* xg = reinterpret_cast<const T*>(a.x) + b * S * a.ld_x;
+  const T* wg = reinterpret_cast<const T*>(a.w) + hd * DH * a.ld_w;
+  const int rb0 = wave * 32;
+  const T* xsrc[4]; T* xdst[4];
+#pragma unroll
+  for (int i = 0; i < 4; ++i) {
+    const int q = lane + 64 * i, r = rb0 + (q >> 3), ch = q & 7;
+    xsrc[i] = xg + (int64_t)(r < S ? r : S - 1) * a.ld_x + ch * 8;
+    xdst[i] = sX + r * DOP_LDS + ch * 8;
+  }
+  const bool extra = TMX == 3 && lone && wave == NW - 1;
+  const int re = 32 * NW + (lane >> 3);
+  const T* const xsrc_e = xg + (int64_t)(re < S ? re : S - 1) * a.ld_x + (lane & 7) * 8;
+  T* const xdst_e = sX + re * DOP_LDS + (lane & 7) * 8;
+  u32x4 xr[4], xe = {0u, 0u, 0u, 0u};
+  auto load_slice = [&](int kc) {
+#pragma unroll
+    for (int i = 0; i < 4; ++i) xr[i] = *reinterpret_cast<const u32x4*>(xsrc[i] + kc * DOP_KC);
+    if (extra) xe = *reinterpret_cast<const u32x4*>(xsrc_e + kc * DOP_KC);
+  };
+  auto store_slice = [&]() {
+#pragma unroll
+    for (int i = 0; i < 4; ++i) *reinterpret_cast<u32x4*>(xdst[i]) = xr[i];
+    if (extra) *reinterpret_cast<u32x4*>(xdst_e) = xe;
+  };
+  load_slice(0);
+  u32x4 qr[2];
+#pragma unroll
+  for (int i = 0; i < 2; ++i) {
+    const int c = tid + i * nthr, row = c / CPR, ch = c % CPR;
+    const bool ok = c < SP * CPR && row < S;
+    const u32x4 v = *reinterpret_cast<const u32x4*>(Qg + (int64_t)(ok ? row : 0) * a.ld_qkv + (ok ? ch : 0) * 8);
+    qr[i] = ok ? v : u32x4{0u, 0u, 0u, 0u};
+  }
+  {
+    const int wpr = D / 8;
+    for (int p = tid; p < DH * wpr; p += nthr) {
+      const int r = p / wpr, ch = p - r * wpr;
+      *reinterpret_cast<u32x4*>(sW + r * LDW + ch * 8) = *reinterpret_cast<const u32x4*>(wg + (int64_t)r * a.ld_w + ch * 8);
+    }
+  }
+  store_slice();
+  __syncthreads();
+  f32x4 acc[TN][TMX];
+#pragma unroll
+  for (int j = 0; j < TN; ++j)
+#pragma unroll
+    for (int i = 0; i < TMX; ++i) acc[j][i] = f32x4{0.f, 0.f, 0.f, 0.f};
+  const int frow = lane & 15, fq = lane >> 4;
+  const T* const fx = sX + (rb0 + frow) * DOP_LDS + 8 * fq;
+  const T* const fxe = sX + (32 * NW + frow) * DOP_LDS + 8 * fq;
+  const T* const fw = sW + frow * LDW + 8 * fq;
+  for (int kc = 0; kc < nch; ++kc) {
+    if (kc + 1 < nch) load_slice(kc + 1);
+#pragma unroll
+    for (int ks = 0; ks < DOP_KC / 32; ++ks) {
+      vec8 xf[2], wf[TN];
+#pragma unroll
+      for (int i = 0; i < 2; ++i) xf[i] = __builtin_bit_cast(vec8, *reinterpret_cast<const u32x4*>(fx + i * 16 * DOP_LDS + 32 * ks));
+#pragma unroll
+      for (int j = 0; j < TN; ++j) wf[j] = __builtin_bit_cast(vec8, *reinterpret_cast<const u32x4*>(fw + j * 16 * LDW + kc * DOP_KC + 32 * ks));
+#pragma unroll
+      for (int j = 0; j < TN; ++j)
+#pragma unroll
+        for (int i = 0; i < 2; ++i) acc[j][i] = Act<T>::mfma16(wf[j], xf[i], acc[j][i]);
+      if constexpr (TMX == 3) {
+        if (extra) {
+          const vec8 xf2 = __builtin_bit_cast(vec8, *reinterpret_cast<const u32x4*>(fxe + 32 * ks));
+#pragma unroll
+          for (int j = 0; j < TN; ++j) acc[j][2] = Act<T>::mfma16(wf[j], xf2, acc[j][2]);
+        }
+      }
+    }
+    wave_lds_fence();
+    if (kc + 1 < nch) store_slice();
+    wave_lds_fence();
+  }
+  __syncthreads();
+#pragma unroll
+  for (int i = 0; i < TMX; ++i) {
+    if (i == 2 && !(lone && wave == NW - 1)) break;
+    const int row = i == 2 ? 32 * NW + frow : rb0 + 16 * i + frow;
+    const bool in = row < S;
+#pragma unroll
+    for (int j = 0; j < TN; ++j) {
+      u32x2 o = {0u, 0u};
+      if (in) {
+        o[0] = (uint32_t)f32_to_bits<T>(acc[j][i][0]) | ((uint32_t)f32_to_bits<T>(acc[j][i][1]) << 16);
+        o[1] = (uint32_t)f32_to_bits<T>(acc[j][i][2]) | ((uint32_t)f32_to_bits<T>(acc[j][i][3]) << 16);
+      }
+      *reinterpret_cast<u32x2*>(bufB + row * LD + 16 * j + 4 * fq) = o;
+      if (i == 2) *reinterpret_cast<u32x2*>(bufB + (row + 16) * LD + 16 * j + 4 * fq) = u32x2{0u, 0u};
+    }
+  }
+#pragma unroll
+  for (int i = 0; i < 2; ++i) {
+    const int c = tid + i * nthr, row = c / CPR, ch = c % CPR;
+    if (c < SP * CPR) *reinterpret_cast<u32x4*>(bufA + row * LD + ch * 8) = qr[i];
+  }
+}
+
+template <typename T, int DH, bool SPARSE, bool PROJ = false>
 __global__ __launch_bounds__(RES_MAX_WAVES<DH> * 64) __attribute__((amdgpu_waves_per_eu(DH == 16 ? ATT16_WAVES : (DH == 64 ? 2 : 4)))) void attn_bwd_res_kernel(AttnArgs a) {
+  static_assert(!PROJ || (!SPARSE && DH <= 32), "the projection prologue: dense, head sizes 16 and 32");
   constexpr int KS = DH / 16, DB = (DH + 31) / 32, LD = LdsLd<DH>::V;
   extern __shared__ __attribute__((aligned(16))) unsigned char att_smem[];
   const int64_t S = a.S;
@@ -1095,8 +1214,18 @@
     vf[s] = glb_row_frag<T>(Vg, a.ld_qkv, wave * 32 + (lane & 31), S, s, lane);
   }
   ATT_STAMP(0);
-  stage_pair<T, DH>(bufA, Qg, a.ld_qkv, S, bufB, dOg, a.ld_dout, do_rows, SP, tid, nthr);
+  if constexpr (PROJ) dout_prologue<T, DH>(a, att_smem, bufA, bufB, Qg, b, hd, NB, lone);
+  else stage_pair<T, DH>(bufA, Qg, a.ld_qkv, S, bufB, dOg, a.ld_dout, do_rows, SP, tid, nthr);
   __syncthreads();
+  if constexpr (PROJ) {
+    if (a.out) {
+      T* const og = reinterpret_cast<T*>(a.out) + b * S * a.ld_out + hd * DH;
+      for (int c = tid; c < (int)S * (DH / 8); c += nthr) {
+        const int row = c / (DH / 8), ch = c % (DH / 8);
+        *reinterpret_cast<u32x4*>(og + (int64_t)row * a.ld_out + ch * 8) = *reinterpret_cast<const u32x4*>(bufB + row * LD + ch * 8);
+      }
+    }
+  }
   ATT_STAMP(1);
   const int nq0 = sparse ? 1 : NBo;
 
@@ -1233,7 +1362,11 @@
 #pragma unroll
   for (int s = 0; s < KS; ++s) {
     qf[s] = glb_row_frag<T>(Qg, a.ld_qkv, wave * 32 + (lane & 31), S, s, lane);
-    dof[s] = glb_row_frag<T>(dOg, a.ld_dout, wave * 32 + (lane & 31), do_rows, s, lane);
+    if constexpr (PROJ) dof[s] = lds_row_frag<T, DH>(bufB, wave * 32, s, lane);
+    else dof[s] = glb_row_frag<T>(dOg, a.ld_dout, wave * 32 + (lane & 31), do_rows, s, lane);
+  }
+  if constexpr (PROJ && DH <= 16) {
+    if (lone && tid < DH) sRed[LONE_RED / 2 + DH + tid] = to_f32(bufB[(S - 1) * LD + tid]);
   }
   __syncthreads();
   stage_pair<T, DH>(bufA, Kg, a.ld_qkv, S, bufB, Vg, a.ld_qkv, S, SP, tid, nthr);
@@ -1247,7 +1380,7 @@
 #pragma unroll
       for (int s = 0; s < KS; ++s) {
         qf[s] = glb_row_frag<T>(Qg, a.ld_qkv, q_lane, S, s, lane);
-        dof[s] = glb_row_frag<T>(dOg, a.ld_dout, q_lane, do_rows, s, lane);
+        if constexpr (!PROJ) dof[s] = glb_row_frag<T>(dOg, a.ld_dout, q_lane, do_rows, s, lane);
       }
     }
     f32x16 acc[DB];
@@ -1278,7 +1411,11 @@
       const int64_t e = S - 1;
       float qe[DH], doe[DH], acc[DH];
 #pragma unroll
-      for (int f = 0; f < DH; ++f) { qe[f] = to_f32(Qg[e * a.ld_qkv + f]); doe[f] = to_f32(dOg[e * a.ld_dout + f]); acc[f] = 0.f; }
+      for (int f = 0; f < DH; ++f) {
+        qe[f] = to_f32(Qg[e * a.ld_qkv + f]); acc[f] = 0.f;
+        if constexpr (PROJ) doe[f] = sRed[LONE_RED / 2 + DH + f];
+        else doe[f] = to_f32(dOg[e * a.ld_dout + f]);
+      }
       for (int k = tid; k < S; k += nthr) {
         const float x = lds_row_dot<T, DH>(bufA + k * LD, qe);
         const float ps = exact ? exact_prob(x, a.scale, sMadd[k], sMax[k], sLogl[k]) * a.scale : fast_exp2(fmaf(x, sSk[k], sCk[k]));
@@ -1406,6 +1543,7 @@
 }
 static size_t res_lds_fwd(int dh, int64_t S, int tiles) { const size_t SP = (size_t)cdiv(S, 32) * 32; return (size_t)tiles * SP * (dh + 8) * 2 + 5 * SP * 4 + LONE_RED * 4; }
 static size_t res_lds_bwd(int dh, int64_t S) { const size_t SP = (size_t)cdiv(S, 32) * 32; return 2 * SP * (dh + 8) * 2 + 6 * SP * 4 + LONE_RED * 4; }
+static size_t res_lds_bwd_proj(int dh, int64_t S, int64_t Dm) { const size_t SP = (size_t)cdiv(S, 32) * 32; return SP * DOP_LDS * 2 + (size_t)dh * (Dm + 8) * 2; }
 static int res_max_waves(int dh) { return dh == 64 ? RES_MAX_WAVES<64> : RES_MAX_WAVES<32>; }
 
 static int attn_check(int64_t B, int64_t S, int64_t H, int64_t dh, int64_t ld, int64_t k_off, int64_t q_off, int64_t v_off) {
@@ -1445,7 +1583,7 @@
 enum { ATT_FWD_RES3 = 0, ATT_FWD_RES2 = 1, ATT_FWD_CHUNKED = 2, ATT_FWD_FUSED = 3, ATT_FWD_STREAM = 4 };
 enum { ATT_BWD_RES = 0, ATT_BWD_STREAM_CHUNKQ = 1, ATT_BWD_STREAM = 2 };
 struct AttnFwdForm { int path, waves; size_t lds; int lone, restage; int64_t grid_stats, grid_out; };
-struct AttnBwdForm { int path, waves; size_t lds; int sparse, lone, dq_chunks, dq_waves; };
+struct AttnBwdForm { int path, waves; size_t lds; int sparse, lone, dq_chunks, dq_waves; int proj; size_t lds_proj; };
 constexpr int ATT_DQ_OBM = 4, ATT_DQ_NW = 8;
 
 static AttnFwdForm attn_fwd_form(int dh, int64_t S, int64_t H, int64_t n_wg, int64_t q_limit, bool fused_call) {
@@ -1498,6 +1636,12 @@
     }
   }
   return f;
+}
+static void attn_bwd_proj_rule(AttnBwdForm& f, int dh, int64_t S, int64_t Dm) {
+  const int NBo = (int)cdiv(S, 32) - f.lone;
+  const size_t need = res_lds_bwd_proj(dh, S, Dm), lds = need > f.lds ? need : f.lds;
+  f.proj = f.path == ATT_BWD_RES && !f.sparse && dh <= 32 && f.waves == NBo && Dm % DOP_KC == 0 && 2 * lds <= 160 * 1024;
+  f.lds_proj = f.proj ? lds : 0;
 }
 
 template <typename T, int DH>
@@ -1548,7 +1692,18 @@
   return MST_ERR_INVALID;
 }
 template <typename T, int DH>
-static int launch_bwd(const AttnArgs& a, const AttnBwdForm& f, hipStream_t s) {
+static int launch_bwd(const AttnArgs& a, const AttnBwdForm& f, hipStream_t s, bool proj = false) {
+  if (proj) {
+    if constexpr (DH <= 32) {
+      static size_t granted = 64 * 1024;
+      if (const int rc = lds_opt_in(reinterpret_cast<const void*>(&attn_bwd_res_kernel<T, DH, false, true>), f.lds_proj, &granted, "attn_bwd_res_kernel (fused projection)")) return rc;
+      hipLaunchKernelGGL((attn_bwd_res_kernel<T, DH, false, true>), dim3((unsigned)(a.B * a.H)), dim3(f.waves * 64), f.lds_proj, s, a);
+      MST_CHECK_LAUNCH("attn_bwd_res_kernel (fused projection)");
+      return MST_OK;
+    }
+    set_error("attention backward: the fused projection has no kernel at head size %d", DH);
+    return MST_ERR_INVALID;
+  }
   if (f.path == ATT_BWD_RES) {
     static size_t granted[2] = {64 * 1024, 64 * 1024};
     const void* fn = f.sparse ? reinterpret_cast<const void*>(&attn_bwd_res_kernel<T, DH, true>)
@@ -1674,8 +1829,9 @@
   int rc = attn_check_bwd(B, S, H, dh, ld_qkv, k_off, q_off, v_off, ld_dout, ld_dqkv);
   if (rc == MST_OK) rc = check_act_dtype(dtype);
   if (rc) return rc;
-  const AttnBwdForm f = attn_bwd_form((int)dh, S, B * H, bwd_q_limit(q_limit, S));
-  const int64_t v[8] = {f.path, f.waves, (int64_t)f.lds, f.sparse, f.lone, f.dq_chunks, f.dq_waves, 0};
+  AttnBwdForm f = attn_bwd_form((int)dh, S, B * H, bwd_q_limit(q_limit, S));
+  attn_bwd_proj_rule(f, (int)dh, S, H * dh);
+  const int64_t v[8] = {f.path, f.waves, (int64_t)f.lds, f.sparse, f.lone, f.dq_chunks, f.dq_waves, f.proj};
   for (int i = 0; i < 8; ++i) form[i] = v[i];
   return MST_OK;
 }
@@ -1744,6 +1900,47 @@
   });
 }
 
+extern "C" int mst_attn_proj_bwd(int dtype, int64_t B, int64_t S, int64_t H, int64_t dh, const void* qkv, int64_t ld_qkv, int64_t k_off,
+                                 int64_t q_off, int64_t v_off, const uint8_t* keymask, const float* lse, const void* dproj, int64_t ld_dproj,
+                                 const void* wt, int64_t ld_wt, void* dout_out, int64_t ld_dout, void* dqkv, int64_t ld_dqkv, float* delta,
+                                 mst_stream_t stream) {
+  int rc = attn_check(B, S, H, dh, ld_qkv, k_off, q_off, v_off);
+  if (rc) return rc;
+  const int64_t Dm = H * dh;
+  MST_CHECK_ARG(qkv && keymask && lse && dproj && wt && dqkv && delta, "mst_attn_proj_bwd: null pointer");
+  MST_CHECK_ARG(ld_dproj % 8 == 0 && ld_dproj >= Dm && ld_wt % 8 == 0 && ld_wt >= Dm && ld_dqkv % 8 == 0 &&
+                (!dout_out || (ld_dout % 8 == 0 && ld_dout >= Dm)), "mst_attn_proj_bwd: bad leading dims");
+  MST_CHECK_ARG(((uintptr_t)dproj % 16 == 0) && ((uintptr_t)wt % 16 == 0) && ((uintptr_t)dout_out % 16 == 0) && ((uintptr_t)qkv % 16 == 0),
+                "mst_attn_proj_bwd: operands must be 16-byte aligned");
+  rc = check_act_dtype(dtype);
+  if (rc) return rc;
+  AttnArgs a = {};
+  a.B = B; a.S = S; a.H = H; a.qkv = qkv; a.ld_qkv = ld_qkv; a.k_off = k_off; a.q_off = q_off; a.v_off = v_off;
+  a.keymask = keymask; a.lse = const_cast<float*>(lse); a.dqkv = dqkv; a.ld_dqkv = ld_dqkv; a.delta = delta;
+  a.q_limit = 0;
+  a.scale = 1.f / sqrtf((float)dh);
+  AttnBwdForm f = attn_bwd_form((int)dh, S, B * H, 0);
+  attn_bwd_proj_rule(f, (int)dh, S, Dm);
+  if (f.proj) {
+    a.x = dproj; a.ld_x = ld_dproj; a.w = wt; a.ld_w = ld_wt; a.Dm = Dm; a.out = dout_out; a.ld_out = ld_dout;
+  } else {
+    MST_CHECK_ARG(dout_out != nullptr, "mst_attn_proj_bwd: this shape runs the GEMM launch first and needs dout_out");
+    mst_gemm_args g = {};
+    g.dtype = dtype; g.M = B * S; g.N = Dm; g.K = Dm;
+    g.A = dproj; g.lda = ld_dproj; g.B = wt; g.ldb = ld_wt; g.C = dout_out; g.ldc = ld_dout; g.alpha = 1.f;
+    rc = mst_gemm_nt(&g, stream);
+    if (rc) return rc;
+    a.dout = dout_out; a.ld_dout = ld_dout;
+  }
+  hipStream_t s = (hipStream_t)stream;
+  return dispatch_act(dtype, [&](auto tag) -> int {
+    typedef decltype(tag) T;
+    if (dh == 16) return launch_bwd<T, 16>(a, f, s, f.proj != 0);
+    if (dh == 32) return launch_bwd<T, 32>(a, f, s, f.proj != 0);
+    return launch_bwd<T, 64>(a, f, s, f.proj != 0);
+  });
+}
+
 extern "C" int mst_attn_decode(int dtype, int64_t B, int64_t H, int64_t dh, int64_t n_keys, int64_t t_max, const void* cache,
                                int64_t ld, int64_t k_off, int64_t q_off, int64_t v_off, int mode, void* out, int64_t ld_out,
                                mst_stream_t stream) {
diff --git a/musicstyletransfer_amd/csrc/runtime.hip b/musicstyletransfer_amd/csrc/runtime.hip
--- a/musicstyletransfer_amd/csrc/runtime.hip
+++ b/musicstyletransfer_amd/csrc/runtime.hip
@@ -14,7 +14,7 @@
 
 using namespace mst;
 
-extern "C" int mst_version(void) { return 112; }
+extern "C" int mst_version(void) { return 113; }
 extern "C" const char* mst_last_error(void) { return g_err; }
 
 #define HIP_TRY(expr)                                             \
diff --git a/musicstyletransfer_amd/engine.py b/musicstyletransfer_amd/engine.py
--- a/musicstyletransfer_amd/engine.py
+++ b/musicstyletransfer_amd/engine.py
@@ -469,7 +469,7 @@
                 resid=None if P.self_resid else t.dh, partials=partials_buf, row_groups=row_groups, **ln1)
 
 
-def row_block_bwd(P, L, t, dy, rows, drop, form, partials, dy_done=False, row_groups=None, tail=None, launch=True):
+def row_block_bwd(P, L, t, dy, rows, drop, form, partials, dy_done=False, row_groups=None, tail=None, launch=True, proj_dgrad=True):
     D, v = P.proj.w.shape[0], rows.view
     if form == "tail":
         o.row_tail_bwd(v(dy), v(L.h2), v(L.h1), v(L.a), L.mean1, L.rstd1, L.mean2, L.rstd2, P.ln1.gamma, P.ln2.gamma, P.ff2.t, P.ff1.t,
@@ -507,7 +507,8 @@
             o.layernorm_bwd(v(L.h1), P.ln1.gamma, L.mean1, L.rstd1, t.dx1, v(t.dh1), P.ln1.dgamma, P.ln1.dbeta, D=D,
                             partials=partials(P.ln1, o.layernorm_bwd_parts(M, D)), **rows.ln, **ln1)
     dproj = t.dh1m if drop.p > 0 else v(t.dh1)
-    o.gemm_nt(dproj, P.proj.t, t.datt, N=D, K=D, c_remap=rows.c_remap)
+    if proj_dgrad:
+        o.gemm_nt(dproj, P.proj.t, t.datt, N=D, K=D, c_remap=rows.c_remap)
     return dff, dproj
 
 
@@ -588,7 +589,8 @@
     return not why
 
 
-Forms = namedtuple("Forms", "tails riders shadows fuse_bce bce_dgrad skip_row0 cls_fold ffn_e ffn_d ln_bwd_e ln_bwd_d sched dec_tail gnorm ema")
+Forms = namedtuple("Forms", "tails riders shadows fuse_bce bce_dgrad skip_row0 cls_fold ffn_e ffn_d ln_bwd_e ln_bwd_d sched dec_tail gnorm ema "
+                            "attn_proj_e attn_proj_d")
 
 
 def check_schedule(kl_warmup_steps=0, kl_cycle_steps=0, kl_free_bits=0.0, lr_warmup_steps=0):
@@ -811,7 +813,11 @@
             ffn_e=o.ffn_fusion_pays(De, 4 * De), ffn_d=ffn_d, ln_bwd_e=o.ln_bwd_fusion_pays(De), ln_bwd_d=ln_bwd_d,
             sched=self.scheduled,
             gnorm=self.clip_global_norm > 0,
-            ema=self.ema_decay > 0)
+            ema=self.ema_decay > 0,
+            attn_proj_e=self._attn_proj(T, cfg.e_heads, De), attn_proj_d=not cfg.d_causal and self._attn_proj(T + 1, cfg.d_heads, Dd))
+
+    def _attn_proj(self, S, H, D):
+        return bool(o.attn_bwd_form(self.adt, self.B, S, H, D // H, 0, D, 2 * D, 3 * D, D, 3 * D, proj=True)["proj"])
 
     def _guard(self):
         fwd, bwd = o.row_tail_barriers(self.cfg.e_model)
@@ -1091,10 +1097,14 @@
         F, P = self.forms, self.store.layer(side, i)
         ffn, ln = (F.ffn_e, F.ln_bwd_e) if side == "encoder" else (F.ffn_d, F.ln_bwd_d)
         in_loss = F.dec_tail and side == "decoder" and i == self.cfg.d_layers - 1
+        proj = F.attn_proj_e if side == "encoder" else F.attn_proj_d
         dff, dproj = row_block_bwd(P, L, t, dy, ALL_ROWS, self._dropout(p, site0), "fused" if ffn else ("ln_fused" if ln else "launches"),
-                                   self._ln_partials, dy_done=dy_done, row_groups=self._row0_groups(side, i), launch=not in_loss)
+                                   self._ln_partials, dy_done=dy_done, row_groups=self._row0_groups(side, i), launch=not in_loss,
+                                   proj_dgrad=not proj)
         if side == "decoder" and self.cfg.d_causal:
             o.attn_causal_bwd(L.qkv, keymask, L.lse, t.datt, t.dqkv, t.delta, self.B, S, H, D // H, 0, D, 2 * D)
+        elif proj:
+            o.attn_proj_bwd(L.qkv, keymask, L.lse, dproj, P.proj.t, t.dqkv, t.delta, self.B, S, H, D // H, 0, D, 2 * D)
         else:
             o.attn_bwd(L.qkv, keymask, L.lse, t.datt, t.dqkv, t.delta, self.B, S, H, D // H, 0, D, 2 * D)
         handed = None
diff --git a/musicstyletransfer_amd/ops.py b/musicstyletransfer_amd/ops.py
--- a/musicstyletransfer_amd/ops.py
+++ b/musicstyletransfer_amd/ops.py
@@ -444,6 +444,11 @@
          ptr(lse), ptr(dout), ld(dout), ptr(dqkv), ld(dqkv), ptr(delta), q_limit, stream())
 
 
+def attn_proj_bwd(qkv, keymask, lse, dproj, Wt, dqkv, delta, B, S, H, dh, k_off, q_off, v_off, dout_out=None):
+    call("mst_attn_proj_bwd", dt(qkv), B, S, H, dh, ptr(qkv), ld(qkv), k_off, q_off, v_off, ptr(keymask), ptr(lse), ptr(dproj), ld(dproj),
+         ptr(Wt), ld(Wt), ptr(dout_out), ld(dout_out) if dout_out is not None else 0, ptr(dqkv), ld(dqkv), ptr(delta), stream())
+
+
 ATTN_FWD_PATHS = ("resident-3", "resident-2", "chunked", "fused", "stream")
 ATTN_BWD_PATHS = ("resident", "stream+chunked-dq", "stream")
 
@@ -454,11 +459,14 @@
     return dict(path=ATTN_FWD_PATHS[form[0]], waves=form[1], lds=form[2], lone=form[3], grid_stats=form[4], grid_out=form[5])
 
 
-def attn_bwd_form(dtype, B, S, H, dh, k_off, q_off, v_off, ld_qkv, ld_dout, ld_dqkv, q_limit=0):
+def attn_bwd_form(dtype, B, S, H, dh, k_off, q_off, v_off, ld_qkv, ld_dout, ld_dqkv, q_limit=0, proj=False):
     form = (C.c_int64 * 8)()
     call("mst_attn_bwd_form", dt(dtype), B, S, H, dh, ld_qkv, k_off, q_off, v_off, ld_dout, ld_dqkv, q_limit, form)
-    return dict(path=ATTN_BWD_PATHS[form[0]], waves=form[1], lds=form[2], sparse=form[3], lone=form[4], dq_chunks=form[5],
-                dq_waves=form[6])
+    d = dict(path=ATTN_BWD_PATHS[form[0]], waves=form[1], lds=form[2], sparse=form[3], lone=form[4], dq_chunks=form[5],
+             dq_waves=form[6])
+    if proj:
+        d["proj"] = form[7]
+    return d
 
 
 def attn_causal_fwd(qkv, keymask, lse, out, B, S, H, dh, k_off, q_off, v_off):
```

After: 26.61 million frames/s (median of 6 runs). 1.02x the previous value.
